# burn-research/OpenMEASURE

Measured on AMD Instinct MI355X. Metric: SPR fit+reconstruct throughput (GB/s snapshot matrix), higher is better.
Workload: dtype f64

## Files before the change

### include/spr_hip.h

```cpp
#ifndef SPR_HIP_H
#define SPR_HIP_H

#include <stddef.h>
#include <stdint.h>

#ifdef __cplusplus
extern "C" {
#endif

#define SPR_OK 0
#define SPR_E_INVALID (-1)
#define SPR_E_UNSUPPORTED (-2)
#define SPR_E_HIP (-3)
#define SPR_E_WORKSPACE (-4)

#define SPR_MAX_M 256
#define SPR_MAX_M_WIDE 512
#define SPR_MAX_R 128
#define SPR_MAX_R_STREAM 256
#define SPR_MAX_R_WIDE 1024

#define SPR_ABI_VERSION 5
int spr_abi_version(void);
const char *spr_last_error(void);
int spr_device_cus(int *out_cus);
int spr_upload_bytes(void *d_dst, const void *h_pinned_src, int64_t n_bytes, void *stream);
int spr_download_bytes(void *h_pinned_dst, const void *d_src, int64_t n_bytes, void *h_pinned_ticket, uint64_t ticket_value,
                       void *stream);
int spr_host_tridiag_vectors(const double *h_d, const double *h_e, int32_t m, const double *h_lam, int32_t r, double *h_Z,
                             int32_t iterations);
int spr_host_eig_top(const double *h_G, int32_t m, int32_t r, double *h_lam, double *h_V, void *fn_dsytrd, void *fn_dsterf,
                     void *fn_dormtr);
int spr_host_svd_top(const double *h_M, int32_t m, int32_t r, double *h_S, double *h_V, void *fn_dgebrd, void *fn_dbdsdc,
                     void *fn_dormbr);

size_t spr_stats_gram_workspace(int32_t m, int32_t n_features);
int spr_stats_gram_f64(const double *d_X, int64_t n_rows, int32_t m, int64_t ldx,
                       int64_t row0, int64_t n_points, int32_t n_features, int32_t center,
                       double *d_rowmean, void *d_workspace, size_t workspace_bytes, void *stream);
int spr_stats_gram_finalize_f64(int64_t n_rows, int32_t m, int64_t row0, int64_t n_points,
                                int32_t n_features, const void *d_workspace, size_t workspace_bytes,
                                double *d_fstats, double *d_gram, int32_t ldg, int32_t origin,
                                void *stream);
size_t spr_rowstats_workspace(int32_t n_features);
int spr_rowstats_f64(const double *d_X, int64_t n_rows, int32_t m, int64_t ldx, int64_t row0,
                     int64_t n_points, int32_t n_features, double *d_rowmean, double *d_fstats,
                     void *d_workspace, size_t workspace_bytes, void *stream);
size_t spr_gram_cross_workspace(int32_t m, int32_t n_features);
int spr_gram_cross_f64(const double *d_X, int64_t n_rows, int32_t m, int64_t ldx, int64_t row0,
                       int64_t n_points, int32_t n_features, int32_t center, double *d_rowmean,
                       double *d_gram, void *d_workspace, size_t workspace_bytes, void *stream);
int spr_rowmean_stats_f64(const double *d_rowmean, int64_t n_rows, int64_t row0, int64_t n_points,
                          int32_t n_features, double *d_fstats, void *d_workspace, size_t workspace_bytes,
                          void *stream);
int spr_gram_cross_pair_f64(const double *d_X, int64_t n_rows, int32_t col_a, int32_t col_b, int32_t w_b,
                            int32_t ldg, int64_t ldx, int64_t row0, int64_t n_points, int32_t n_features,
                            int32_t center, double *d_rowmean, double *d_gram, void *d_workspace,
                            size_t workspace_bytes, void *stream);

int32_t spr_spectrum_max_m(void);
int spr_spectrum_f64(const double *d_gram, const double *d_fstats_all, int32_t n_ranks,
                     int32_t n_features, int32_t m, int32_t scale_code, int32_t r, double *d_feat,
                     double *d_scale, double *d_inv_scale, double *d_lam, double *d_S, double *d_expvar,
                     double *d_V, double *d_W, double *d_Ar, double *d_info, void *stream);

int spr_gram_combine_f64(const double *d_gram, const double *d_fstats_all, int32_t n_ranks,
                         int32_t n_features, int32_t m, int32_t scale_code, double *d_G, double *d_feat,
                         double *d_scale, double *d_inv_scale, void *stream);

int spr_stats_gram_shifted_f64(const double *d_X, int64_t n_rows, int32_t m, int64_t ldx, int64_t row0,
                               int64_t n_points, int32_t n_features, const double *d_shift, double *d_rowsum,
                               void *d_workspace, size_t workspace_bytes, void *stream);
int spr_gram_shift_finish_f64(double *d_rowmean, const double *d_rowsum_b, int64_t n_rows, int32_t w_a, int32_t m,
                              double *d_gram, int32_t n_features, void *stream);

int spr_project_f64(const double *d_X, int64_t n_rows, int32_t m, int64_t ldx,
                    int64_t row0, int64_t n_points, int32_t n_features, int32_t center,
                    const double *d_inv_scale, const double *d_rowmean, const double *d_W, int32_t r,
                    double *d_Ur, int64_t ldu, int32_t accumulate, void *stream);

size_t spr_project_stream_workspace(int32_t m, int32_t r, int32_t x_is_f32);
int spr_project_stream_f64(const double *d_X, int64_t n_rows, int32_t m, int64_t ldx, int64_t row0,
                           int64_t n_points, int32_t n_features, int32_t center, const double *d_inv_scale,
                           const double *d_rowmean, const double *d_W, int32_t r, double *d_Ur, int64_t ldu,
                           void *d_workspace, size_t workspace_bytes, void *stream);

int32_t spr_project_norms_supported(int32_t m, int32_t r, int64_t n_rows, int64_t ldx, const void *d_X,
                                    int32_t x_is_f32);
int spr_project_norms_f64(const double *d_X, int64_t n_rows, int32_t m, int64_t ldx, int64_t row0,
                          int64_t n_points, int32_t n_features, int32_t center, const double *d_inv_scale,
                          const double *d_rowmean, const double *d_W, int32_t r, double *d_Ur, int64_t ldu,
                          double *d_rownorm2, void *stream);
int spr_project_stream_norms_f64(const double *d_X, int64_t n_rows, int32_t m, int64_t ldx, int64_t row0,
                                 int64_t n_points, int32_t n_features, int32_t center, const double *d_inv_scale,
                                 const double *d_rowmean, const double *d_W, int32_t r, double *d_Ur, int64_t ldu,
                                 double *d_rownorm2, void *d_workspace, size_t workspace_bytes, void *stream);

int spr_scale_rows_f64(const double *d_X, int64_t n_rows, int32_t m, int64_t ldx, int64_t row0,
                       int64_t n_points, int32_t n_features, const double *d_rowmean,
                       const double *d_inv_scale, double *d_X0, int64_t ldo, void *stream);
int spr_unscale_f64(const double *d_x0, int64_t n_rows, int64_t row0, int64_t n_points,
                    int32_t n_features, const double *d_rowmean, const double *d_scale,
                    const double *d_rowscale, double *d_x, void *stream);

size_t spr_feature_minmax_workspace(int32_t n_features);
int spr_feature_minmax_f64(const double *d_X, int64_t n_rows, int32_t m, int64_t ldx, int64_t row0,
                           int64_t n_points, int32_t n_features, double *d_minmax,
                           void *d_workspace, size_t workspace_bytes, void *stream);

int spr_feature_digit_hist_f64(const double *d_X, int64_t n_rows, int32_t m, int64_t ldx, int64_t row0,
                               int64_t n_points, int32_t n_features, const uint64_t *d_prefix, int32_t shift,
                               int32_t bits, int32_t two_targets, uint64_t *d_hist, void *stream);

size_t spr_colsums_workspace(int32_t m, int32_t n_features);
int spr_colsums_f64(const double *d_X, int64_t n_rows, int32_t m, int64_t ldx, int64_t row0,
                    int64_t n_points, int32_t n_features, const double *d_rowmean, double *d_out,
                    void *d_workspace, size_t workspace_bytes, void *stream);
int spr_fill_feature_f64(double *d_out, int64_t n_rows, int64_t row0, int64_t n_points, int32_t n_features,
                         const double *d_values, void *stream);

int spr_reconstruct_f64(const double *d_Ur, int64_t n_rows, int32_t r, int64_t ldu,
                        int64_t row0, int64_t n_points, int32_t n_features,
                        const double *d_rowmean, const double *d_scale, const double *d_rowscale,
                        const double *d_A, int32_t n_p, double *d_Xrec, int64_t ldo,
                        void *stream);
size_t spr_bound_sweep_workspace(int32_t n_p, int32_t n_features);
int spr_bound_sweep_f64(const double *d_Ur, int64_t n_rows, int32_t r, int64_t ldu, int64_t row0, int64_t n_points,
                        int32_t n_features, const double *d_rowmean, const double *d_scale, const double *d_limits,
                        const double *d_clamp, const double *d_G, int32_t n_p, double tol, int32_t k, double *d_out,
                        void *d_workspace, size_t workspace_bytes, void *stream);
int spr_bound_sweep_u32(const float *d_Ur, int64_t n_rows, int32_t r, int64_t ldu, int64_t row0, int64_t n_points,
                        int32_t n_features, const double *d_rowmean, const double *d_scale, const double *d_limits,
                        const double *d_clamp, const double *d_G, int32_t n_p, double tol, int32_t k, double *d_out,
                        void *d_workspace, size_t workspace_bytes, void *stream);
size_t spr_bound_sweep_batch_workspace(int32_t n_p, int32_t n_features);
int spr_bound_sweep_batch_f64(const double *d_Ur, int64_t n_rows, int32_t r, int64_t ldu, int64_t row0, int64_t n_points,
                              int32_t n_features, const double *d_rowmean, const double *d_scale, const double *d_limits,
                              const double *d_clamp, const double *d_G, int32_t n_p, double tol, int32_t k, double *d_out,
                              void *d_workspace, size_t workspace_bytes, void *stream);
int spr_bound_sweep_batch_u32(const float *d_Ur, int64_t n_rows, int32_t r, int64_t ldu, int64_t row0, int64_t n_points,
                              int32_t n_features, const double *d_rowmean, const double *d_scale, const double *d_limits,
                              const double *d_clamp, const double *d_G, int32_t n_p, double tol, int32_t k, double *d_out,
                              void *d_workspace, size_t workspace_bytes, void *stream);
size_t spr_encode_workspace(int32_t r, int32_t k, int32_t n_features);
int spr_encode_f64(const double *d_Ur, int64_t n_rows, int32_t r, int64_t ldu, const double *d_X, int32_t k, int64_t ldx,
                   int64_t row0, int64_t n_points, int32_t n_features, const double *d_rowmean, const double *d_scale,
                   double *d_A, void *d_workspace, size_t workspace_bytes, void *stream);
int spr_encode_x32(const double *d_Ur, int64_t n_rows, int32_t r, int64_t ldu, const float *d_X, int32_t k, int64_t ldx,
                   int64_t row0, int64_t n_points, int32_t n_features, const double *d_rowmean, const double *d_scale,
                   double *d_A, void *d_workspace, size_t workspace_bytes, void *stream);
int spr_encode_u32(const float *d_Ur, int64_t n_rows, int32_t r, int64_t ldu, const double *d_X, int32_t k, int64_t ldx,
                   int64_t row0, int64_t n_points, int32_t n_features, const double *d_rowmean, const double *d_scale,
                   double *d_A, void *d_workspace, size_t workspace_bytes, void *stream);
int spr_encode_x32_u32(const float *d_Ur, int64_t n_rows, int32_t r, int64_t ldu, const float *d_X, int32_t k, int64_t ldx,
                       int64_t row0, int64_t n_points, int32_t n_features, const double *d_rowmean, const double *d_scale,
                       double *d_A, void *d_workspace, size_t workspace_bytes, void *stream);
size_t spr_field_error_workspace(int32_t k, int32_t n_features);
int spr_field_error_f64(const double *d_Ur, int64_t n_rows, int32_t r, int64_t ldu, int64_t row0, int64_t n_points,
                        int32_t n_features, const double *d_rowmean, const double *d_scale, const double *d_A, int32_t k,
                        const double *d_Xtrue, int64_t ldx, double *d_out, void *d_workspace, size_t workspace_bytes,
                        void *stream);
int spr_field_error_x32(const double *d_Ur, int64_t n_rows, int32_t r, int64_t ldu, int64_t row0, int64_t n_points,
                        int32_t n_features, const double *d_rowmean, const double *d_scale, const double *d_A, int32_t k,
                        const float *d_Xtrue, int64_t ldx, double *d_out, void *d_workspace, size_t workspace_bytes,
                        void *stream);
int spr_field_error_u32(const float *d_Ur, int64_t n_rows, int32_t r, int64_t ldu, int64_t row0, int64_t n_points,
                        int32_t n_features, const double *d_rowmean, const double *d_scale, const double *d_A, int32_t k,
                        const double *d_Xtrue, int64_t ldx, double *d_out, void *d_workspace, size_t workspace_bytes,
                        void *stream);
int spr_field_error_x32_u32(const float *d_Ur, int64_t n_rows, int32_t r, int64_t ldu, int64_t row0, int64_t n_points,
                            int32_t n_features, const double *d_rowmean, const double *d_scale, const double *d_A, int32_t k,
                            const float *d_Xtrue, int64_t ldx, double *d_out, void *d_workspace, size_t workspace_bytes,
                            void *stream);
size_t spr_gappy_normal_workspace(int32_t r, int32_t k, int32_t n_features);
int spr_gappy_normal_f64(const double *d_Ur, int64_t n_rows, int32_t r, int64_t ldu, const double *d_X, int32_t k,
                         int64_t ldx, int64_t row0, int64_t n_points, int32_t n_features, const double *d_rowmean,
                         const double *d_scale, const uint8_t *d_mask, int64_t ldm, double *d_H, double *d_B,
                         double *d_nobs, void *d_workspace, size_t workspace_bytes, void *stream);
int spr_gappy_normal_x32(const double *d_Ur, int64_t n_rows, int32_t r, int64_t ldu, const float *d_X, int32_t k,
                         int64_t ldx, int64_t row0, int64_t n_points, int32_t n_features, const double *d_rowmean,
                         const double *d_scale, const uint8_t *d_mask, int64_t ldm, double *d_H, double *d_B,
                         double *d_nobs, void *d_workspace, size_t workspace_bytes, void *stream);
int spr_gappy_normal_u32(const float *d_Ur, int64_t n_rows, int32_t r, int64_t ldu, const double *d_X, int32_t k,
                         int64_t ldx, int64_t row0, int64_t n_points, int32_t n_features, const double *d_rowmean,
                         const double *d_scale, const uint8_t *d_mask, int64_t ldm, double *d_H, double *d_B,
                         double *d_nobs, void *d_workspace, size_t workspace_bytes, void *stream);
int spr_gappy_normal_x32_u32(const float *d_Ur, int64_t n_rows, int32_t r, int64_t ldu, const float *d_X, int32_t k,
                             int64_t ldx, int64_t row0, int64_t n_points, int32_t n_features, const double *d_rowmean,
                             const double *d_scale, const uint8_t *d_mask, int64_t ldm, double *d_H, double *d_B,
                             double *d_nobs, void *d_workspace, size_t workspace_bytes, void *stream);
size_t spr_gappy_fill_workspace(void);
int spr_gappy_rowfill_f64(double *d_X, int64_t n_rows, int32_t m, int64_t ldx, int64_t row0, const uint8_t *d_mask,
                          int64_t ldm, double *d_out, void *d_workspace, size_t workspace_bytes, void *stream);
int spr_gappy_rowfill_x32(float *d_X, int64_t n_rows, int32_t m, int64_t ldx, int64_t row0, const uint8_t *d_mask,
                          int64_t ldm, double *d_out, void *d_workspace, size_t workspace_bytes, void *stream);
int spr_gappy_fill_f64(const double *d_Ur, int64_t n_rows, int32_t r, int64_t ldu, double *d_X, int32_t m, int64_t ldx,
                       int64_t row0, int64_t n_points, int32_t n_features, const double *d_rowmean, const double *d_scale,
                       const double *d_A, const uint8_t *d_mask, int64_t ldm, double *d_out, void *d_workspace,
                       size_t workspace_bytes, void *stream);
int spr_gappy_fill_x32(const double *d_Ur, int64_t n_rows, int32_t r, int64_t ldu, float *d_X, int32_t m, int64_t ldx,
                       int64_t row0, int64_t n_points, int32_t n_features, const double *d_rowmean, const double *d_scale,
                       const double *d_A, const uint8_t *d_mask, int64_t ldm, double *d_out, void *d_workspace,
                       size_t workspace_bytes, void *stream);
int spr_gappy_fill_u32(const float *d_Ur, int64_t n_rows, int32_t r, int64_t ldu, double *d_X, int32_t m, int64_t ldx,
                       int64_t row0, int64_t n_points, int32_t n_features, const double *d_rowmean, const double *d_scale,
                       const double *d_A, const uint8_t *d_mask, int64_t ldm, double *d_out, void *d_workspace,
                       size_t workspace_bytes, void *stream);
int spr_gappy_fill_x32_u32(const float *d_Ur, int64_t n_rows, int32_t r, int64_t ldu, float *d_X, int32_t m, int64_t ldx,
                           int64_t row0, int64_t n_points, int32_t n_features, const double *d_rowmean,
                           const double *d_scale, const double *d_A, const uint8_t *d_mask, int64_t ldm, double *d_out,
                           void *d_workspace, size_t workspace_bytes, void *stream);
int spr_field_std_diag_f64(const double *d_Ur, int64_t n_rows, int32_t r, int64_t ldu, int64_t row0, int64_t n_points,
                           int32_t n_features, const double *d_scale, const double *d_rowscale, const double *d_S,
                           int32_t k, double *d_out, int64_t ldo, void *stream);
int spr_field_std_diag_u32(const float *d_Ur, int64_t n_rows, int32_t r, int64_t ldu, int64_t row0, int64_t n_points,
                           int32_t n_features, const double *d_scale, const double *d_rowscale, const double *d_S,
                           int32_t k, double *d_out, int64_t ldo, void *stream);
int spr_field_std_factor_f64(const double *d_Ur, int64_t n_rows, int32_t r, int64_t ldu, int64_t row0, int64_t n_points,
                             int32_t n_features, const double *d_scale, const double *d_rowscale, const double *d_L,
                             int32_t k, int32_t q, double *d_out, int64_t ldo, void *stream);
int spr_field_std_factor_u32(const float *d_Ur, int64_t n_rows, int32_t r, int64_t ldu, int64_t row0, int64_t n_points,
                             int32_t n_features, const double *d_scale, const double *d_rowscale, const double *d_L,
                             int32_t k, int32_t q, double *d_out, int64_t ldo, void *stream);
#define SPR_GP_MAX_M 800
#define SPR_GP_MATERN52 0
#define SPR_GP_MATERN32 1
#define SPR_GP_MATERN12 2
#define SPR_GP_RBF 3
size_t spr_gp_workspace(int32_t m, int32_t r);
int spr_gp_train_f64(const double *d_P0, int32_t m, int32_t d, int64_t ldp, const double *d_Y, int32_t r, int64_t ldy,
                     int32_t kernel, double *d_raw, double lr, int32_t max_iter, double tol, double *d_Kinv, double *d_alpha,
                     double *d_info, double *d_trace, void *d_workspace, size_t workspace_bytes, void *stream);
int spr_gp_predict_f64(const double *d_P0, int32_t m, int32_t d, int64_t ldp, const double *d_Pstar, int32_t n_p,
                       int64_t ldps, int32_t kernel, const double *d_raw, int32_t r, const double *d_Kinv,
                       const double *d_alpha, double *d_mean, double *d_var, void *stream);
#define SPR_GP_MAX_D 8
#define SPR_GP_FLAG_ARD 1
#define SPR_GP_FLAG_SCALE 2
size_t spr_gp_workspace_ard(int32_t m, int32_t d, int32_t r);
int spr_gp_train_ard_f64(const double *d_P0, int32_t m, int32_t d, int64_t ldp, const double *d_Y, int32_t r, int64_t ldy,
                         int32_t kernel, int32_t flags, double *d_raw, double lr, int32_t max_iter, double tol,
                         double *d_Kinv, double *d_alpha, double *d_info, double *d_trace, void *d_workspace,
                         size_t workspace_bytes, void *stream);
int spr_gp_predict_ard_f64(const double *d_P0, int32_t m, int32_t d, int64_t ldp, const double *d_Pstar, int32_t n_p,
                           int64_t ldps, int32_t kernel, int32_t flags, const double *d_raw, int32_t r, const double *d_Kinv,
                           const double *d_alpha, double *d_mean, double *d_var, void *stream);
int spr_field_unstage_f64(const double *d_stage, int32_t world, int32_t n_p, int64_t n_loc, double *d_out, int64_t ldo,
                          void *stream);
int spr_field_unstage_blocks_f64(const double *d_stage, int32_t world, int32_t n_p, int64_t n_max, const int64_t *d_layout,
                                 double *d_out, int64_t ldo, void *stream);

size_t spr_p2p_handle_bytes(void);
int spr_p2p_alloc(size_t n_bytes, int32_t kind, void **d_ptr, void *h_handle);
int spr_p2p_free(void *d_ptr);
int spr_p2p_open(const void *h_handle, void **d_mapped);
int spr_p2p_close(void *d_mapped);
int spr_p2p_device_id(char *h_buf, int32_t n_buf);
int spr_p2p_peer_access(const char *h_bus_id, int32_t *h_can);
int spr_p2p_signal(void *d_flag, uint64_t value, void *stream);
int spr_p2p_wait(void *d_flag, uint64_t value, void *stream);
int spr_p2p_flags_set(void *const *d_flags, int32_t n, uint64_t value, void *stream);
int spr_p2p_flags_wait(void *const *d_flags, int32_t n, uint64_t value, double timeout_s, void *d_status, void *stream);
int spr_p2p_copy(void *d_dst, const void *d_src, int64_t n_bytes, void *stream);
uint64_t spr_p2p_poison_bit(void);
int spr_field_gather_p2p(const double *d_field, int64_t ldo, int32_t n_p, int64_t first, int64_t n_loc, int32_t n_peers,
                         void *const *d_peer_field, void *const *d_release_flag, uint64_t release_value,
                         double release_timeout_s, void *const *d_peer_arrive_flag, uint64_t arrive_value,
                         void *const *d_pushed_flag, void *const *streams, void *d_status, void *d_ready_flag,
                         uint64_t ready_value);
int spr_field_gather_p2p_join(void *const *d_flags, int32_t n_flags, uint64_t arrive_value, double timeout_s, void *d_status,
                              void *stream);
int spr_field_gather_p2p_release(void *const *d_peer_release_flag, int32_t n_peers, uint64_t value, void *stream);

size_t spr_comm_unique_id_bytes(void);
int spr_comm_unique_id(void *h_id);
int spr_comm_init(const void *h_id, int32_t rank, int32_t world, void **comm);
int spr_comm_destroy(void *comm);
int spr_comm_info(void *comm, int32_t *rank, int32_t *world);
const char *spr_comm_library(void);
int spr_allreduce_f64(void *comm, double *d_buf, int64_t count, void *stream);
int spr_allreduce_i64(void *comm, int64_t *d_buf, int64_t count, void *stream);
int spr_allgather(void *comm, const void *d_send, void *d_recv, int64_t bytes_per_rank, void *stream);
size_t spr_fit_gram_pass_buffer(int32_t m, int32_t n_features, int32_t world);
size_t spr_fit_gram_pass_workspace(int32_t m, int32_t n_features, int64_t n_rows);
int spr_fit_gram_pass(void *comm, const void *d_X, int32_t x_is_f32, int64_t n_rows, int32_t m, int64_t ldx, int64_t row0,
                      int64_t n_points, int32_t n_features, int32_t scale_code, double *d_rowmean, double *d_buf,
                      size_t buf_bytes, double *d_G, double *d_feat, double *d_scale, double *d_inv_scale, void *d_workspace,
                      size_t workspace_bytes, void *stream);

#define SPR_QR_REC_LEN(r) ((r) + 3)
size_t spr_qr_workspace(int64_t n_rows);
size_t spr_qr_workspace_r(int64_t n_rows, int32_t r);
int32_t spr_qr_batch(void);
int spr_mask_rows_f64(double *d_Ur, int64_t n_rows, int32_t r, int64_t ldu,
                      const uint8_t *d_mask, void *stream);
int spr_qr_init_f64(const double *d_Ur, int64_t n_rows, int32_t r, int64_t ldu,
                    int64_t row0, double *d_nrm, double *d_rec, double *d_tau,
                    void *d_workspace, size_t workspace_bytes, void *stream);
int spr_qr_init_norms_f64(const double *d_Ur, int64_t n_rows, int32_t r, int64_t ldu, int64_t row0,
                          const double *d_nrm0, double *d_nrm, double *d_rec, double *d_tau,
                          void *d_workspace, size_t workspace_bytes, void *stream);
int spr_qr_step_f64(int64_t n_rows, int32_t r, int32_t step, const double *d_recs, int32_t n_rec,
                    const double *d_taus, int32_t n_tau, int32_t first, double *d_Q,
                    int64_t *d_piv, double *d_gap, double *d_ok, double *d_rec,
                    const double *d_xyz, int32_t xyz_dim, int64_t n_points, double d_min,
                    void *d_workspace, size_t workspace_bytes, void *stream);
int spr_qr_steps_f64(int64_t n_rows, int32_t r, int32_t step0, int32_t n_steps, int32_t first_exact,
                     const double *d_tau, double *d_Q, int64_t *d_piv, double *d_gap, double *d_ok, double *d_rec,
                     const double *d_xyz, int32_t xyz_dim, int64_t n_points, double d_min,
                     void *d_workspace, size_t workspace_bytes, void *stream);
int32_t spr_qr_epoch_supported(int32_t r, int64_t ldu, const void *d_Ur, int32_t u_is_f32, int64_t n_rows);
int32_t spr_qr_epoch_max_directions(int32_t r);
size_t spr_qr_pool_workspace(void);
int spr_qr_pool_build(const double *d_nrm_e, int64_t n_rows, double theta, int32_t *d_pool, int64_t cap,
                      int32_t *d_pool_n, void *d_workspace, size_t workspace_bytes, void *stream);
int spr_qr_epoch_sweep_f64(const double *d_Ur, int64_t n_rows, int32_t r, int64_t ldu, int64_t row0,
                           const double *d_Q, const int64_t *d_piv, int32_t j_e, int32_t j, int32_t j_mark,
                           double *d_nrm_e, double *d_nrm, const int32_t *d_pool, const int32_t *d_pool_n,
                           int64_t pool_n_host, double tau_floor, double *d_rec, double *d_tau,
                           void *d_workspace, size_t workspace_bytes, void *stream);
int spr_qr_exclude_f64(double *d_nrm, int64_t n_rows, int64_t row0, int64_t n_points,
                       const uint8_t *d_mask, const double *d_xyz, int32_t xyz_dim,
                       const int64_t *d_piv, int32_t nq, double d_min, void *stream);
int spr_qr_refresh_f64(const double *d_Ur, int64_t n_rows, int32_t r, int64_t ldu, int64_t row0,
                       const double *d_Q, const int64_t *d_piv, int32_t j0, int32_t nq,
                       double *d_nrm, double *d_rec, double *d_tau,
                       void *d_workspace, size_t workspace_bytes, void *stream);

int spr_measure_csr_f64(const int64_t *d_indptr, const int64_t *d_indices,
                        const double *d_vals, int32_t s, const double *d_Ur,
                        int64_t n_rows, int32_t r, int64_t ldu, int64_t row0,
                        const double *d_rowmean, const double *d_scale, int64_t n_points,
                        int32_t n_features, double *d_Theta, double *d_cnt, double *d_scl,
                        void *stream);

int spr_solve_ols_f64(const double *d_Theta, int32_t s, int32_t r, const double *d_cnt,
                      const double *d_scale, int32_t n_features, const double *d_y,
                      int32_t n_p, double *d_Ar, double *d_Ar_sigma, double *d_y0,
                      double *d_info, void *stream);

size_t spr_solve_ols_workspace(int32_t s, int32_t r, int32_t n_p);
int spr_solve_ols_wide_f64(const double *d_Theta, int32_t s, int32_t r, const double *d_cnt,
                           const double *d_scale, int32_t n_features, const double *d_y, int32_t n_p,
                           double *d_Ar, double *d_Ar_sigma, double *d_y0, double *d_info, void *d_workspace,
                           size_t workspace_bytes, void *stream);

int spr_solve_pinv_f64(const double *d_Theta, int32_t s, int32_t r, const double *d_cnt, int32_t s_cnt,
                       const double *d_scale, int32_t n_features, const double *d_y, int32_t n_p,
                       double rcond, double *d_Ar, double *d_Ar_sigma, double *d_y0, double *d_info,
                       void *stream);

size_t spr_solve_pinv_workspace(int32_t r, int32_t n_p);
int spr_solve_pinv_wide_f64(const double *d_Theta, int32_t s, int32_t r, const double *d_cnt, int32_t s_cnt,
                            const double *d_scale, int32_t n_features, const double *d_y, int32_t n_p,
                            double rcond, double *d_Ar, double *d_Ar_sigma, double *d_y0, double *d_info,
                            void *d_workspace, size_t workspace_bytes, void *stream);

size_t spr_assimilate_workspace(int32_t s, int32_t r, int32_t q, int32_t n_p);
int spr_assimilate_f64(const double *d_Theta, int32_t s, int32_t r, const double *d_cnt, const double *d_scale,
                       int32_t n_features, const double *d_y, int32_t n_p, const double *d_a0, const double *d_sigma,
                       const double *d_factor, int32_t q, double *d_Ar, double *d_Ar_std, double *d_F, double *d_z,
                       double *d_info, void *d_workspace, size_t workspace_bytes, void *stream);

int spr_synth_f64(double *d_X, int64_t n_rows, int32_t ncols, int64_t ldx, int64_t row0,
                  int64_t n_points, int32_t col0, const double *d_R, int32_t k, int32_t ldr,
                  double eps, uint64_t seed, void *stream);
int spr_synth_gather_f64(const int64_t *d_rows, int32_t n, int64_t n_points, int32_t col,
                         const double *d_R, int32_t k, int32_t ldr, double eps,
                         uint64_t seed, double *d_out, void *stream);

int spr_stats_gram_x32(const float *d_X, int64_t n_rows, int32_t m, int64_t ldx, int64_t row0,
                       int64_t n_points, int32_t n_features, int32_t center, double *d_rowmean,
                       void *d_workspace, size_t workspace_bytes, void *stream);
int spr_rowstats_x32(const float *d_X, int64_t n_rows, int32_t m, int64_t ldx, int64_t row0,
                     int64_t n_points, int32_t n_features, double *d_rowmean, double *d_fstats,
                     void *d_workspace, size_t workspace_bytes, void *stream);
int spr_gram_cross_x32(const float *d_X, int64_t n_rows, int32_t m, int64_t ldx, int64_t row0,
                       int64_t n_points, int32_t n_features, int32_t center, double *d_rowmean,
                       double *d_gram, void *d_workspace, size_t workspace_bytes, void *stream);
int spr_gram_cross_pair_x32(const float *d_X, int64_t n_rows, int32_t col_a, int32_t col_b, int32_t w_b,
                            int32_t ldg, int64_t ldx, int64_t row0, int64_t n_points, int32_t n_features,
                            int32_t center, double *d_rowmean, double *d_gram, void *d_workspace,
                            size_t workspace_bytes, void *stream);
int spr_project_x32(const float *d_X, int64_t n_rows, int32_t m, int64_t ldx, int64_t row0,
                    int64_t n_points, int32_t n_features, int32_t center, const double *d_inv_scale,
                    const double *d_rowmean, const double *d_W, int32_t r, float *d_Ur, int64_t ldu,
                    int32_t accumulate, void *stream);
int spr_project_x32_f64out(const float *d_X, int64_t n_rows, int32_t m, int64_t ldx, int64_t row0,
                           int64_t n_points, int32_t n_features, int32_t center, const double *d_inv_scale,
                           const double *d_rowmean, const double *d_W, int32_t r, double *d_Ur, int64_t ldu,
                           int32_t accumulate, void *stream);
int spr_project_x32_acc(const float *d_X, int64_t n_rows, int32_t m, int64_t ldx, int64_t row0,
                        int64_t n_points, int32_t n_features, int32_t center, const double *d_inv_scale,
                        const double *d_rowmean, const double *d_W, int32_t r, const double *d_acc_in,
                        int64_t lda, float *d_Ur, int64_t ldu, void *stream);
int spr_project_stream_x32(const float *d_X, int64_t n_rows, int32_t m, int64_t ldx, int64_t row0,
                           int64_t n_points, int32_t n_features, int32_t center, const double *d_inv_scale,
                           const double *d_rowmean, const double *d_W, int32_t r, float *d_Ur, int64_t ldu,
                           void *d_workspace, size_t workspace_bytes, void *stream);
int spr_project_stream_x32_f64out(const float *d_X, int64_t n_rows, int32_t m, int64_t ldx, int64_t row0,
                                  int64_t n_points, int32_t n_features, int32_t center, const double *d_inv_scale,
                                  const double *d_rowmean, const double *d_W, int32_t r, double *d_Ur, int64_t ldu,
                                  void *d_workspace, size_t workspace_bytes, void *stream);
int spr_project_norms_x32(const float *d_X, int64_t n_rows, int32_t m, int64_t ldx, int64_t row0,
                          int64_t n_points, int32_t n_features, int32_t center, const double *d_inv_scale,
                          const double *d_rowmean, const double *d_W, int32_t r, float *d_Ur, int64_t ldu,
                          double *d_rownorm2, void *stream);
int spr_project_norms_x32_f64out(const float *d_X, int64_t n_rows, int32_t m, int64_t ldx, int64_t row0,
                                 int64_t n_points, int32_t n_features, int32_t center, const double *d_inv_scale,
                                 const double *d_rowmean, const double *d_W, int32_t r, double *d_Ur, int64_t ldu,
                                 double *d_rownorm2, void *stream);
int spr_project_stream_norms_x32(const float *d_X, int64_t n_rows, int32_t m, int64_t ldx, int64_t row0,
                                 int64_t n_points, int32_t n_features, int32_t center, const double *d_inv_scale,
                                 const double *d_rowmean, const double *d_W, int32_t r, float *d_Ur, int64_t ldu,
                                 double *d_rownorm2, void *d_workspace, size_t workspace_bytes, void *stream);
int spr_project_stream_norms_x32_f64out(const float *d_X, int64_t n_rows, int32_t m, int64_t ldx, int64_t row0,
                                        int64_t n_points, int32_t n_features, int32_t center,
                                        const double *d_inv_scale, const double *d_rowmean, const double *d_W,
                                        int32_t r, double *d_Ur, int64_t ldu, double *d_rownorm2, void *d_workspace,
                                        size_t workspace_bytes, void *stream);
int spr_stats_gram_shifted_x32(const float *d_X, int64_t n_rows, int32_t m, int64_t ldx, int64_t row0,
                               int64_t n_points, int32_t n_features, const double *d_shift, double *d_rowsum,
                               void *d_workspace, size_t workspace_bytes, void *stream);
int spr_scale_rows_x32(const float *d_X, int64_t n_rows, int32_t m, int64_t ldx, int64_t row0,
                       int64_t n_points, int32_t n_features, const double *d_rowmean,
                       const double *d_inv_scale, double *d_X0, int64_t ldo, void *stream);
int spr_feature_minmax_x32(const float *d_X, int64_t n_rows, int32_t m, int64_t ldx, int64_t row0,
                           int64_t n_points, int32_t n_features, double *d_minmax,
                           void *d_workspace, size_t workspace_bytes, void *stream);
int spr_colsums_x32(const float *d_X, int64_t n_rows, int32_t m, int64_t ldx, int64_t row0,
                    int64_t n_points, int32_t n_features, const double *d_rowmean, double *d_out,
                    void *d_workspace, size_t workspace_bytes, void *stream);
int spr_feature_digit_hist_x32(const float *d_X, int64_t n_rows, int32_t m, int64_t ldx, int64_t row0,
                               int64_t n_points, int32_t n_features, const uint64_t *d_prefix, int32_t shift,
                               int32_t bits, int32_t two_targets, uint64_t *d_hist, void *stream);
int spr_synth_f32(float *d_X, int64_t n_rows, int32_t ncols, int64_t ldx, int64_t row0,
                  int64_t n_points, int32_t col0, const double *d_R, int32_t k, int32_t ldr,
                  double eps, uint64_t seed, void *stream);
int spr_reconstruct_u32(const float *d_Ur, int64_t n_rows, int32_t r, int64_t ldu, int64_t row0,
                        int64_t n_points, int32_t n_features, const double *d_rowmean,
                        const double *d_scale, const double *d_rowscale, const double *d_A, int32_t n_p,
                        double *d_Xrec, int64_t ldo, void *stream);
int spr_mask_rows_u32(float *d_Ur, int64_t n_rows, int32_t r, int64_t ldu,
                      const uint8_t *d_mask, void *stream);
int spr_qr_init_u32(const float *d_Ur, int64_t n_rows, int32_t r, int64_t ldu,
                    int64_t row0, double *d_nrm, double *d_rec, double *d_tau,
                    void *d_workspace, size_t workspace_bytes, void *stream);
int spr_qr_init_norms_u32(const float *d_Ur, int64_t n_rows, int32_t r, int64_t ldu, int64_t row0,
                          const double *d_nrm0, double *d_nrm, double *d_rec, double *d_tau,
                          void *d_workspace, size_t workspace_bytes, void *stream);
int spr_qr_epoch_sweep_u32(const float *d_Ur, int64_t n_rows, int32_t r, int64_t ldu, int64_t row0,
                           const double *d_Q, const int64_t *d_piv, int32_t j_e, int32_t j, int32_t j_mark,
                           double *d_nrm_e, double *d_nrm, const int32_t *d_pool, const int32_t *d_pool_n,
                           int64_t pool_n_host, double tau_floor, double *d_rec, double *d_tau,
                           void *d_workspace, size_t workspace_bytes, void *stream);
int spr_qr_refresh_u32(const float *d_Ur, int64_t n_rows, int32_t r, int64_t ldu, int64_t row0,
                       const double *d_Q, const int64_t *d_piv, int32_t j0, int32_t nq,
                       double *d_nrm, double *d_rec, double *d_tau,
                       void *d_workspace, size_t workspace_bytes, void *stream);
int spr_measure_csr_u32(const int64_t *d_indptr, const int64_t *d_indices, const double *d_vals,
                        int32_t s, const float *d_Ur, int64_t n_rows, int32_t r, int64_t ldu,
                        int64_t row0, const double *d_rowmean, const double *d_scale, int64_t n_points,
                        int32_t n_features, double *d_Theta, double *d_cnt, double *d_scl, void *stream);

#ifdef __cplusplus
}
#endif
#endif
```

### openmeasure_amd/_lib.py

```python
from __future__ import annotations

import ctypes as C
import os

_HERE = os.path.dirname(os.path.abspath(__file__))
LIB_PATH = os.environ.get('SPR_HIP_LIBRARY') or os.path.join(_HERE, 'libspr_hip.so')

SPR_ABI_VERSION = 5
SPR_MAX_M = 256
SPR_MAX_M_WIDE = 512
SPR_MAX_R = 128
SPR_MAX_R_STREAM = 256
SPR_MAX_R_WIDE = 1024
SPR_GP_MAX_M = 800
SPR_GP_MAX_D = 8

_i32, _i64, _u64, _sz = C.c_int32, C.c_int64, C.c_uint64, C.c_size_t
_p = C.c_void_p
_dbl = C.c_double

PROTOTYPES = {
    'spr_abi_version': (C.c_int, []),
    'spr_last_error': (C.c_char_p, []),
    'spr_device_cus': (C.c_int, [C.POINTER(C.c_int)]),
    'spr_upload_bytes': (C.c_int, [_p, _p, _i64, _p]),
    'spr_download_bytes': (C.c_int, [_p, _p, _i64, _p, _u64, _p]),
    'spr_host_tridiag_vectors': (C.c_int, [_p, _p, _i32, _p, _i32, _p, _i32]),
    'spr_host_eig_top': (C.c_int, [_p, _i32, _i32, _p, _p, _p, _p, _p]),
    'spr_host_svd_top': (C.c_int, [_p, _i32, _i32, _p, _p, _p, _p, _p]),
    'spr_stats_gram_workspace': (_sz, [_i32, _i32]),
    'spr_stats_gram_f64': (C.c_int, [_p, _i64, _i32, _i64, _i64, _i64, _i32, _i32, _p, _p, _sz, _p]),
    'spr_stats_gram_finalize_f64': (C.c_int, [_i64, _i32, _i64, _i64, _i32, _p, _sz, _p, _p, _i32, _i32, _p]),
    'spr_stats_gram_shifted_f64': (C.c_int, [_p, _i64, _i32, _i64, _i64, _i64, _i32, _p, _p, _p, _sz, _p]),
    'spr_gram_shift_finish_f64': (C.c_int, [_p, _p, _i64, _i32, _i32, _p, _i32, _p]),
    'spr_rowstats_workspace': (_sz, [_i32]),
    'spr_rowstats_f64': (C.c_int, [_p, _i64, _i32, _i64, _i64, _i64, _i32, _p, _p, _p, _sz, _p]),
    'spr_gram_cross_workspace': (_sz, [_i32, _i32]),
    'spr_gram_cross_f64': (C.c_int, [_p, _i64, _i32, _i64, _i64, _i64, _i32, _i32, _p, _p, _p, _sz, _p]),
    'spr_gram_cross_pair_f64': (C.c_int, [_p, _i64, _i32, _i32, _i32, _i32, _i64, _i64, _i64, _i32, _i32, _p, _p, _p, _sz, _p]),
    'spr_rowmean_stats_f64': (C.c_int, [_p, _i64, _i64, _i64, _i32, _p, _p, _sz, _p]),
    'spr_spectrum_max_m': (_i32, []),
    'spr_spectrum_f64': (C.c_int, [_p, _p, _i32, _i32, _i32, _i32, _i32, _p, _p, _p, _p, _p, _p, _p, _p, _p, _p, _p]),
    'spr_gram_combine_f64': (C.c_int, [_p, _p, _i32, _i32, _i32, _i32, _p, _p, _p, _p, _p]),
    'spr_project_f64': (C.c_int, [_p, _i64, _i32, _i64, _i64, _i64, _i32, _i32, _p, _p, _p, _i32, _p, _i64, _i32, _p]),
    'spr_project_norms_supported': (_i32, [_i32, _i32, _i64, _i64, _p, _i32]),
    'spr_project_norms_f64': (C.c_int, [_p, _i64, _i32, _i64, _i64, _i64, _i32, _i32, _p, _p, _p, _i32, _p, _i64, _p, _p]),
    'spr_project_stream_norms_f64': (C.c_int, [_p, _i64, _i32, _i64, _i64, _i64, _i32, _i32, _p, _p, _p, _i32, _p, _i64, _p, _p, _sz, _p]),
    'spr_project_stream_workspace': (_sz, [_i32, _i32, _i32]),
    'spr_project_stream_f64': (C.c_int, [_p, _i64, _i32, _i64, _i64, _i64, _i32, _i32, _p, _p, _p, _i32, _p, _i64, _p, _sz, _p]),
    'spr_scale_rows_f64': (C.c_int, [_p, _i64, _i32, _i64, _i64, _i64, _i32, _p, _p, _p, _i64, _p]),
    'spr_unscale_f64': (C.c_int, [_p, _i64, _i64, _i64, _i32, _p, _p, _p, _p, _p]),
    'spr_feature_minmax_workspace': (_sz, [_i32]),
    'spr_feature_minmax_f64': (C.c_int, [_p, _i64, _i32, _i64, _i64, _i64, _i32, _p, _p, _sz, _p]),
    'spr_feature_digit_hist_f64': (C.c_int, [_p, _i64, _i32, _i64, _i64, _i64, _i32, _p, _i32, _i32, _i32, _p, _p]),
    'spr_colsums_workspace': (_sz, [_i32, _i32]),
    'spr_colsums_f64': (C.c_int, [_p, _i64, _i32, _i64, _i64, _i64, _i32, _p, _p, _p, _sz, _p]),
    'spr_fill_feature_f64': (C.c_int, [_p, _i64, _i64, _i64, _i32, _p, _p]),
    'spr_reconstruct_f64': (C.c_int, [_p, _i64, _i32, _i64, _i64, _i64, _i32, _p, _p, _p, _p, _i32, _p, _i64, _p]),
    'spr_bound_sweep_workspace': (_sz, [_i32, _i32]),
    'spr_bound_sweep_f64': (C.c_int, [_p, _i64, _i32, _i64, _i64, _i64, _i32, _p, _p, _p, _p, _p, _i32, _dbl, _i32, _p, _p, _sz, _p]),
    'spr_bound_sweep_batch_workspace': (_sz, [_i32, _i32]),
    'spr_bound_sweep_batch_f64': (C.c_int, [_p, _i64, _i32, _i64, _i64, _i64, _i32, _p, _p, _p, _p, _p, _i32, _dbl, _i32, _p, _p, _sz, _p]),
    'spr_encode_workspace': (_sz, [_i32, _i32, _i32]),
    'spr_encode_f64': (C.c_int, [_p, _i64, _i32, _i64, _p, _i32, _i64, _i64, _i64, _i32, _p, _p, _p, _p, _sz, _p]),
    'spr_field_error_workspace': (_sz, [_i32, _i32]),
    'spr_field_error_f64': (C.c_int, [_p, _i64, _i32, _i64, _i64, _i64, _i32, _p, _p, _p, _i32, _p, _i64, _p, _p, _sz, _p]),
    'spr_gappy_normal_workspace': (_sz, [_i32, _i32, _i32]),
    'spr_gappy_normal_f64': (C.c_int, [_p, _i64, _i32, _i64, _p, _i32, _i64, _i64, _i64, _i32, _p, _p, _p, _i64, _p, _p, _p, _p, _sz, _p]),
    'spr_gappy_fill_workspace': (_sz, []),
    'spr_gappy_rowfill_f64': (C.c_int, [_p, _i64, _i32, _i64, _i64, _p, _i64, _p, _p, _sz, _p]),
    'spr_gappy_fill_f64': (C.c_int, [_p, _i64, _i32, _i64, _p, _i32, _i64, _i64, _i64, _i32, _p, _p, _p, _p, _i64, _p, _p, _sz, _p]),
    'spr_field_std_diag_f64': (C.c_int, [_p, _i64, _i32, _i64, _i64, _i64, _i32, _p, _p, _p, _i32, _p, _i64, _p]),
    'spr_field_std_factor_f64': (C.c_int, [_p, _i64, _i32, _i64, _i64, _i64, _i32, _p, _p, _p, _i32, _i32, _p, _i64, _p]),
    'spr_gp_workspace': (_sz, [_i32, _i32]),
    'spr_gp_train_f64': (C.c_int, [_p, _i32, _i32, _i64, _p, _i32, _i64, _i32, _p, _dbl, _i32, _dbl, _p, _p, _p, _p, _p, _sz, _p]),
    'spr_gp_predict_f64': (C.c_int, [_p, _i32, _i32, _i64, _p, _i32, _i64, _i32, _p, _i32, _p, _p, _p, _p, _p]),
    'spr_gp_workspace_ard': (_sz, [_i32, _i32, _i32]),
    'spr_gp_train_ard_f64': (C.c_int, [_p, _i32, _i32, _i64, _p, _i32, _i64, _i32, _i32, _p, _dbl, _i32, _dbl, _p, _p, _p, _p, _p, _sz, _p]),
    'spr_gp_predict_ard_f64': (C.c_int, [_p, _i32, _i32, _i64, _p, _i32, _i64, _i32, _i32, _p, _i32, _p, _p, _p, _p, _p]),
    'spr_field_unstage_f64': (C.c_int, [_p, _i32, _i32, _i64, _p, _i64, _p]),
    'spr_field_unstage_blocks_f64': (C.c_int, [_p, _i32, _i32, _i64, _p, _p, _i64, _p]),
    'spr_p2p_handle_bytes': (_sz, []),
    'spr_p2p_alloc': (C.c_int, [_sz, _i32, _p, _p]),
    'spr_p2p_free': (C.c_int, [_p]),
    'spr_p2p_open': (C.c_int, [_p, _p]),
    'spr_p2p_close': (C.c_int, [_p]),
    'spr_p2p_device_id': (C.c_int, [_p, _i32]),
    'spr_p2p_peer_access': (C.c_int, [_p, _p]),
    'spr_p2p_signal': (C.c_int, [_p, _u64, _p]),
    'spr_p2p_wait': (C.c_int, [_p, _u64, _p]),
    'spr_p2p_flags_set': (C.c_int, [_p, _i32, _u64, _p]),
    'spr_p2p_flags_wait': (C.c_int, [_p, _i32, _u64, _dbl, _p, _p]),
    'spr_p2p_copy': (C.c_int, [_p, _p, _i64, _p]),
    'spr_p2p_poison_bit': (_u64, []),
    'spr_field_gather_p2p': (C.c_int, [_p, _i64, _i32, _i64, _i64, _i32, _p, _p, _u64, _dbl, _p, _u64, _p, _p, _p, _p, _u64]),
    'spr_field_gather_p2p_join': (C.c_int, [_p, _i32, _u64, _dbl, _p, _p]),
    'spr_field_gather_p2p_release': (C.c_int, [_p, _i32, _u64, _p]),
    'spr_qr_workspace': (_sz, [_i64]),
    'spr_qr_workspace_r': (_sz, [_i64, _i32]),
    'spr_qr_batch': (_i32, []),
    'spr_mask_rows_f64': (C.c_int, [_p, _i64, _i32, _i64, _p, _p]),
    'spr_qr_init_f64': (C.c_int, [_p, _i64, _i32, _i64, _i64, _p, _p, _p, _p, _sz, _p]),
    'spr_qr_init_norms_f64': (C.c_int, [_p, _i64, _i32, _i64, _i64, _p, _p, _p, _p, _p, _sz, _p]),
    'spr_qr_step_f64': (C.c_int, [_i64, _i32, _i32, _p, _i32, _p, _i32, _i32, _p, _p, _p, _p, _p, _p, _i32, _i64, _dbl, _p, _sz, _p]),
    'spr_qr_steps_f64': (C.c_int, [_i64, _i32, _i32, _i32, _i32, _p, _p, _p, _p, _p, _p, _p, _i32, _i64, _dbl, _p, _sz, _p]),
    'spr_qr_epoch_supported': (_i32, [_i32, _i64, _p, _i32, _i64]),
    'spr_qr_epoch_max_directions': (_i32, [_i32]),
    'spr_qr_pool_workspace': (_sz, []),
    'spr_qr_pool_build': (C.c_int, [_p, _i64, _dbl, _p, _i64, _p, _p, _sz, _p]),
    'spr_qr_epoch_sweep_f64': (C.c_int, [_p, _i64, _i32, _i64, _i64, _p, _p, _i32, _i32, _i32, _p, _p, _p, _p, _i64, _dbl, _p, _p, _p, _sz, _p]),
    'spr_qr_exclude_f64': (C.c_int, [_p, _i64, _i64, _i64, _p, _p, _i32, _p, _i32, _dbl, _p]),
    'spr_qr_refresh_f64': (C.c_int, [_p, _i64, _i32, _i64, _i64, _p, _p, _i32, _i32, _p, _p, _p, _p, _sz, _p]),
    'spr_measure_csr_f64': (C.c_int, [_p, _p, _p, _i32, _p, _i64, _i32, _i64, _i64, _p, _p, _i64, _i32, _p, _p, _p, _p]),
    'spr_solve_ols_f64': (C.c_int, [_p, _i32, _i32, _p, _p, _i32, _p, _i32, _p, _p, _p, _p, _p]),
    'spr_solve_ols_workspace': (_sz, [_i32, _i32, _i32]),
    'spr_solve_ols_wide_f64': (C.c_int, [_p, _i32, _i32, _p, _p, _i32, _p, _i32, _p, _p, _p, _p, _p, _sz, _p]),
    'spr_solve_pinv_f64': (C.c_int, [_p, _i32, _i32, _p, _i32, _p, _i32, _p, _i32, _dbl, _p, _p, _p, _p, _p]),
    'spr_solve_pinv_workspace': (_sz, [_i32, _i32]),
    'spr_solve_pinv_wide_f64': (C.c_int, [_p, _i32, _i32, _p, _i32, _p, _i32, _p, _i32, _dbl, _p, _p, _p, _p, _p, _sz, _p]),
    'spr_assimilate_workspace': (_sz, [_i32, _i32, _i32, _i32]),
    'spr_assimilate_f64': (C.c_int, [_p, _i32, _i32, _p, _p, _i32, _p, _i32, _p, _p, _p, _i32, _p, _p, _p, _p, _p, _p, _sz, _p]),
    'spr_comm_unique_id_bytes': (_sz, []),
    'spr_comm_unique_id': (C.c_int, [_p]),
    'spr_comm_init': (C.c_int, [_p, _i32, _i32, _p]),
    'spr_comm_destroy': (C.c_int, [_p]),
    'spr_comm_info': (C.c_int, [_p, _p, _p]),
    'spr_comm_library': (C.c_char_p, []),
    'spr_allreduce_f64': (C.c_int, [_p, _p, _i64, _p]),
    'spr_allreduce_i64': (C.c_int, [_p, _p, _i64, _p]),
    'spr_allgather': (C.c_int, [_p, _p, _p, _i64, _p]),
    'spr_fit_gram_pass_buffer': (_sz, [_i32, _i32, _i32]),
    'spr_fit_gram_pass_workspace': (_sz, [_i32, _i32, _i64]),
    'spr_fit_gram_pass': (C.c_int, [_p, _p, _i32, _i64, _i32, _i64, _i64, _i64, _i32, _i32, _p, _p, _sz, _p, _p, _p, _p, _p, _sz, _p]),
    'spr_synth_f64': (C.c_int, [_p, _i64, _i32, _i64, _i64, _i64, _i32, _p, _i32, _i32, _dbl, _u64, _p]),
    'spr_synth_gather_f64': (C.c_int, [_p, _i32, _i64, _i32, _p, _i32, _i32, _dbl, _u64, _p, _p]),
}

_lib = None


class SprError(RuntimeError):
    """A libspr_hip.so call returned a negative status."""


PROTOTYPES['spr_project_x32_acc'] = (C.c_int, [_p, _i64, _i32, _i64, _i64, _i64, _i32, _i32, _p, _p, _p, _i32, _p, _i64, _p, _i64, _p])

for _f64, _x32 in (('spr_stats_gram_f64', 'spr_stats_gram_x32'), ('spr_stats_gram_shifted_f64', 'spr_stats_gram_shifted_x32'), ('spr_rowstats_f64', 'spr_rowstats_x32'),
                   ('spr_gram_cross_f64', 'spr_gram_cross_x32'), ('spr_gram_cross_pair_f64', 'spr_gram_cross_pair_x32'), ('spr_project_f64', 'spr_project_x32'),
                   ('spr_project_f64', 'spr_project_x32_f64out'),
                   ('spr_project_stream_f64', 'spr_project_stream_x32'),
                   ('spr_project_stream_f64', 'spr_project_stream_x32_f64out'),
                   ('spr_project_norms_f64', 'spr_project_norms_x32'),
                   ('spr_project_norms_f64', 'spr_project_norms_x32_f64out'),
                   ('spr_project_stream_norms_f64', 'spr_project_stream_norms_x32'),
                   ('spr_project_stream_norms_f64', 'spr_project_stream_norms_x32_f64out'),
                   ('spr_qr_init_norms_f64', 'spr_qr_init_norms_u32'),
                   ('spr_qr_epoch_sweep_f64', 'spr_qr_epoch_sweep_u32'),
                   ('spr_scale_rows_f64', 'spr_scale_rows_x32'), ('spr_feature_minmax_f64', 'spr_feature_minmax_x32'),
                   ('spr_colsums_f64', 'spr_colsums_x32'), ('spr_feature_digit_hist_f64', 'spr_feature_digit_hist_x32'),
                   ('spr_synth_f64', 'spr_synth_f32'), ('spr_reconstruct_f64', 'spr_reconstruct_u32'),
                   ('spr_bound_sweep_f64', 'spr_bound_sweep_u32'),
                   ('spr_bound_sweep_batch_f64', 'spr_bound_sweep_batch_u32'),
                   ('spr_encode_f64', 'spr_encode_x32'), ('spr_encode_f64', 'spr_encode_u32'),
                   ('spr_encode_f64', 'spr_encode_x32_u32'),
                   ('spr_field_error_f64', 'spr_field_error_x32'), ('spr_field_error_f64', 'spr_field_error_u32'),
                   ('spr_field_error_f64', 'spr_field_error_x32_u32'),
                   ('spr_gappy_normal_f64', 'spr_gappy_normal_x32'), ('spr_gappy_normal_f64', 'spr_gappy_normal_u32'),
                   ('spr_gappy_normal_f64', 'spr_gappy_normal_x32_u32'),
                   ('spr_gappy_rowfill_f64', 'spr_gappy_rowfill_x32'),
                   ('spr_gappy_fill_f64', 'spr_gappy_fill_x32'), ('spr_gappy_fill_f64', 'spr_gappy_fill_u32'),
                   ('spr_gappy_fill_f64', 'spr_gappy_fill_x32_u32'),
                   ('spr_field_std_diag_f64', 'spr_field_std_diag_u32'),
                   ('spr_field_std_factor_f64', 'spr_field_std_factor_u32'),
                   ('spr_mask_rows_f64', 'spr_mask_rows_u32'), ('spr_qr_init_f64', 'spr_qr_init_u32'),
                   ('spr_qr_refresh_f64', 'spr_qr_refresh_u32'), ('spr_measure_csr_f64', 'spr_measure_csr_u32')):
    PROTOTYPES[_x32] = PROTOTYPES[_f64]


def load():
    global _lib
    if _lib is not None:
        return _lib
    if not os.path.exists(LIB_PATH):
        raise RuntimeError(
            f'{LIB_PATH} is missing: build it with `make -C openmeasure_amd/csrc` '
            '(or __graft_entry__.build()). There is no CPU fallback for the SPR kernels.')
    import torch
    lib = C.CDLL(LIB_PATH, mode=C.RTLD_GLOBAL)
    for name, (res, args) in PROTOTYPES.items():
        fn = getattr(lib, name)
        fn.restype = res
        fn.argtypes = args
    have = lib.spr_abi_version()
    if have != SPR_ABI_VERSION:
        raise RuntimeError(f'{LIB_PATH} reports ABI version {have}, this binding was written for {SPR_ABI_VERSION}: '
                           'rebuild the library (make -C openmeasure_amd/csrc) or use the matching package')
    _lib = lib
    return lib


def check(rc, what=''):
    if rc == 0:
        return
    msg = load().spr_last_error().decode('utf-8', 'replace')
    kinds = {-1: ValueError, -2: NotImplementedError, -3: SprError, -4: MemoryError}
    raise kinds.get(rc, SprError)(f'{what or "libspr_hip"} failed (status {rc}): {msg}')
```

### openmeasure_amd/csrc/common.hpp

```cpp
#pragma once
#include <hip/hip_runtime.h>
#include <stdint.h>
#include <stdio.h>

#include "spr_hip.h"

typedef double f64x4 __attribute__((ext_vector_type(4)));
typedef double f64x2 __attribute__((ext_vector_type(2)));

void spr_set_error(const char *fmt, ...);

#define SPR_REQUIRE(cond, code, ...)      \
  do {                                    \
    if (!(cond)) {                        \
      spr_set_error(__VA_ARGS__);         \
      return (code);                      \
    }                                     \
  } while (0)

#define SPR_HIP_TRY(expr)                                                          \
  do {                                                                             \
    hipError_t e__ = (expr);                                                       \
    if (e__ != hipSuccess) {                                                       \
      spr_set_error("%s failed: %s (%s:%d)", #expr, hipGetErrorString(e__),       \
                    __FILE__, __LINE__);                                           \
      return SPR_E_HIP;                                                            \
    }                                                                              \
  } while (0)

#define SPR_LAUNCH_CHECK()                                                         \
  do {                                                                             \
    hipError_t e__ = hipGetLastError();                                            \
    if (e__ != hipSuccess) {                                                       \
      spr_set_error("kernel launch failed: %s (%s:%d)", hipGetErrorString(e__),   \
                    __FILE__, __LINE__);                                           \
      return SPR_E_HIP;                                                            \
    }                                                                              \
  } while (0)

int spr_cached_cus();

struct SegPlan {
  int64_t row0, n_rows, n_points;
  int32_t n_features;
  int32_t total_wg;
  int32_t chunk_rows;
};

__host__ __device__ inline void seg_range(const SegPlan &p, int f, int64_t &lo, int64_t &hi) {
  int64_t glo = (int64_t)f * p.n_points, ghi = glo + p.n_points;
  if (glo < p.row0) glo = p.row0;
  if (ghi > p.row0 + p.n_rows) ghi = p.row0 + p.n_rows;
  if (ghi < glo) ghi = glo;
  lo = glo - p.row0;
  hi = ghi - p.row0;
}

__host__ __device__ inline int seg_wgs(const SegPlan &p, int64_t rows) {
  if (rows <= 0) return 0;
  int64_t w = rows * (int64_t)p.total_wg / p.n_rows;
  int64_t chunks = (rows + p.chunk_rows - 1) / p.chunk_rows;
  if (w > chunks) w = chunks;
  if (w < 1) w = 1;
  return (int)w;
}

__host__ __device__ inline int seg_first_feature(const SegPlan &p) { return (int)(p.row0 / p.n_points); }
__host__ __device__ inline int seg_last_feature(const SegPlan &p) {
  int64_t f = (p.row0 + p.n_rows - 1) / p.n_points;
  if (f > p.n_features - 1) f = p.n_features - 1;
  return (int)f;
}

inline int seg_total_wgs(const SegPlan &p) {
  int tot = 0;
  for (int f = seg_first_feature(p); f <= seg_last_feature(p); ++f) {
    int64_t lo, hi;
    seg_range(p, f, lo, hi);
    tot += seg_wgs(p, hi - lo);
  }
  return tot;
}

__device__ inline bool seg_locate(const SegPlan &p, int b, int &f, int &wl, int &wpf, int &base,
                                  int64_t &lo, int64_t &hi) {
  int acc = 0;
  int f1 = seg_last_feature(p);
  for (int ff = seg_first_feature(p); ff <= f1; ++ff) {
    seg_range(p, ff, lo, hi);
    int w = seg_wgs(p, hi - lo);
    if (b < acc + w) {
      f = ff; wl = b - acc; wpf = w; base = acc;
      return true;
    }
    acc += w;
  }
  return false;
}

template <int CTRL>
__device__ inline double dpp_f64(double v) {
  union { double d; int i[2]; } a, b;
  a.d = v;
  b.i[0] = __builtin_amdgcn_update_dpp(0, a.i[0], CTRL, 0xF, 0xF, true);
  b.i[1] = __builtin_amdgcn_update_dpp(0, a.i[1], CTRL, 0xF, 0xF, true);
  return b.d;
}

template <int WIDTH>
__device__ inline double group_sum_t(double v) {
  if (WIDTH >= 2) v += dpp_f64<0xB1>(v);
  if (WIDTH >= 4) v += dpp_f64<0x4E>(v);
  if (WIDTH >= 8) v += dpp_f64<0x141>(v);
  if (WIDTH >= 16) v += dpp_f64<0x140>(v);
  if (WIDTH >= 32) v += __shfl_xor(v, 16, 64);
  if (WIDTH >= 64) v += __shfl_xor(v, 32, 64);
  return v;
}

__device__ inline double group_sum(double v, int width) {
  for (int o = width >> 1; o > 0; o >>= 1) v += __shfl_xor(v, o, 64);
  return v;
}

constexpr int spr_pow2_divisor_le64(int n) {
  int p = 1;
  while (p < 64 && n % (2 * p) == 0) p *= 2;
  return p;
}

inline int spr_round_mt(int m) {
  static const int sup[] = {1, 2, 3, 4, 6, 8, 12, 16};
  int need = (m + 15) / 16;
  for (int s : sup)
    if (s >= need) return s;
  return -1;
}
```

### openmeasure_amd/csrc/launch.hpp

```cpp
#pragma once
#include "common.hpp"

inline int spr_cus_or_default() {
  const int cus = spr_cached_cus();
  return cus > 0 ? cus : 256;
}

inline bool spr_layout_ok(int64_t row0, int64_t n_rows, int64_t n_points, int32_t n_features) {
  return n_points > 0 && n_features > 0 && row0 >= 0 && row0 + n_rows <= n_points * (int64_t)n_features;
}
#define SPR_REQUIRE_LAYOUT(name, row0, n_rows, n_points, n_features) \
  SPR_REQUIRE(spr_layout_ok(row0, n_rows, n_points, n_features), SPR_E_INVALID, "%s: bad feature layout", name)

inline SegPlan spr_make_plan(int64_t row0, int64_t n_rows, int64_t n_points, int32_t n_features, int32_t chunk_rows) {
  SegPlan plan;
  plan.row0 = row0; plan.n_rows = n_rows; plan.n_points = n_points; plan.n_features = n_features;
  plan.total_wg = 0; plan.chunk_rows = chunk_rows;
  return plan;
}

inline int spr_plan_grid(SegPlan &plan, int per_cu, int chunk_rows) {
  plan.total_wg = per_cu * spr_cus_or_default();
  plan.chunk_rows = chunk_rows;
  return seg_total_wgs(plan);
}

inline int spr_plan_grid(SegPlan &plan, int per_cu) { return spr_plan_grid(plan, per_cu, plan.chunk_rows); }

constexpr int spr_panel_per_cu(int mtr) { return mtr <= 1 ? 6 : mtr == 2 ? 4 : mtr == 3 ? 3 : mtr == 4 ? 2 : 1; }

#define SPR_REQUIRE_GRID(name, grid, max_slots) \
  SPR_REQUIRE((grid) > 0 && (grid) <= (max_slots), SPR_E_INVALID, "%s: grid of %d exceeds the workspace", name, grid)

template <typename T>
inline bool spr_pair_aligned(const T *p, int64_t cols, int64_t ld) {
  return (cols % 2 == 0) && (ld % 2 == 0) && ((reinterpret_cast<uintptr_t>(p) & (2 * sizeof(T) - 1)) == 0);
}

inline bool spr_rows_aligned16(const void *p, size_t row_bytes) {
  return row_bytes % 16 == 0 && (reinterpret_cast<uintptr_t>(p) & 15) == 0;
}

inline int spr_load_mode(bool pair_aligned, int r, int mtr) { return pair_aligned ? (r == 16 * mtr ? 2 : 1) : 0; }

#define SPR_RUNG_(N, ...) \
  case N: {               \
    constexpr int RUNG = N; \
    __VA_ARGS__;          \
  } break;
#define SPR_NO_RUNG_(name, r) \
  default: SPR_REQUIRE(false, SPR_E_UNSUPPORTED, "%s: no kernel for the padded width of r = %d", name, (int)(r));

#define SPR_DISPATCH_MT(sel, name, r, ...)                   \
  switch (sel) {                                                                                                  \
    SPR_RUNG_(1, __VA_ARGS__) SPR_RUNG_(2, __VA_ARGS__) SPR_RUNG_(3, __VA_ARGS__) SPR_RUNG_(4, __VA_ARGS__)       \
    SPR_RUNG_(6, __VA_ARGS__) SPR_RUNG_(8, __VA_ARGS__) SPR_NO_RUNG_(name, r)                                     \
  }
#define SPR_DISPATCH_POW2(sel, name, r, ...)                         \
  switch (sel) {                                                                                                  \
    SPR_RUNG_(1, __VA_ARGS__) SPR_RUNG_(2, __VA_ARGS__) SPR_RUNG_(4, __VA_ARGS__) SPR_RUNG_(8, __VA_ARGS__)       \
    SPR_NO_RUNG_(name, r)                                                                                         \
  }
#define SPR_DISPATCH_1TO8(sel, name, r, ...)                                 \
  switch (sel) {                                                                                                  \
    SPR_RUNG_(1, __VA_ARGS__) SPR_RUNG_(2, __VA_ARGS__) SPR_RUNG_(3, __VA_ARGS__) SPR_RUNG_(4, __VA_ARGS__)       \
    SPR_RUNG_(5, __VA_ARGS__) SPR_RUNG_(6, __VA_ARGS__) SPR_RUNG_(7, __VA_ARGS__) SPR_RUNG_(8, __VA_ARGS__)       \
    SPR_NO_RUNG_(name, r)                                                                                         \
  }

#define SPR_ENTRY(NAME, PARAMS, IMPL, ...) \
  extern "C" int NAME PARAMS { return IMPL(#NAME, __VA_ARGS__); }
```

### openmeasure_amd/csrc/project_ws.hip

```cpp
#include <type_traits>

#include "rowtile.hpp"
#include "launch.hpp"

namespace {

#ifndef WS_ABLATE
#define WS_ABLATE 0
#endif
constexpr int WS_WAVES = 8;
constexpr int WS_ROWS = 16 * WS_WAVES;

template <int RT> struct WsLds { static constexpr int NC = 16 * RT, LDW = NC; static_assert(RT % 2 == 0, "column tiles come in pairs"); };

template <typename TX> struct WsPiece;
template <> struct WsPiece<double> { f64x2 a, b; };
template <> struct WsPiece<float> { float x, y, z, w; };

template <int VEC, typename TX>
__device__ inline WsPiece<TX> ws_load(const TX *__restrict__ rp, int col0, int m) {
  WsPiece<TX> p;
  if constexpr (std::is_same<TX, double>::value) {
    if (VEC) {
      p.a = *reinterpret_cast<const f64x2 *>(rp + col0);
      p.b = *reinterpret_cast<const f64x2 *>(rp + col0 + 2);
    } else {
      p.a.x = rp[col0 < m ? col0 : 0];         p.a.y = rp[col0 + 1 < m ? col0 + 1 : 0];
      p.b.x = rp[col0 + 2 < m ? col0 + 2 : 0]; p.b.y = rp[col0 + 3 < m ? col0 + 3 : 0];
    }
  } else {
    if (VEC) {
      const float4 v = *reinterpret_cast<const float4 *>(rp + col0);
      p.x = v.x; p.y = v.y; p.z = v.z; p.w = v.w;
    } else {
      p.x = rp[col0 < m ? col0 : 0];         p.y = rp[col0 + 1 < m ? col0 + 1 : 0];
      p.z = rp[col0 + 2 < m ? col0 + 2 : 0]; p.w = rp[col0 + 3 < m ? col0 + 3 : 0];
    }
  }
  return p;
}

template <typename TX>
__device__ inline double ws_elem(const WsPiece<TX> &p, int t) {
  if constexpr (std::is_same<TX, double>::value) return t == 0 ? p.a.x : t == 1 ? p.a.y : t == 2 ? p.b.x : p.b.y;
  else return (double)(t == 0 ? p.x : t == 1 ? p.y : t == 2 ? p.z : p.w);
}

template <int MT, int RT, int VEC, typename TX, typename TU, bool NRM>
__global__ __launch_bounds__(WS_WAVES * 64) void project_ws_kernel(
    const TX *__restrict__ X, int64_t ldx, int m, int center_i, SegPlan plan, const double *__restrict__ inv_scale,
    const double *__restrict__ rowmean, const double *__restrict__ W, int r, TU *__restrict__ Ur, int64_t ldu,
    double *__restrict__ nrm2) {
  constexpr int K = 16 * MT, NJ = MT;
  constexpr int NC = WsLds<RT>::NC, LDW = WsLds<RT>::LDW;
  __shared__ double Wl[K * LDW];

  int f, wl, wpf, base;
  int64_t lo, hi;
  if (!seg_locate(plan, blockIdx.x, f, wl, wpf, base, lo, hi)) return;

  const int lane = threadIdx.x & 63;
  const int wave = __builtin_amdgcn_readfirstlane(threadIdx.x >> 6);
  const int li = lane & 15, kk = lane >> 4;
  const double isc = inv_scale[f];

  for (int e = threadIdx.x; e < K * NC; e += WS_WAVES * 64) {
    const int k = e / NC, c = e - k * NC;
    Wl[k * LDW + (c >> 5) * 32 + (c & 15) * 2 + ((c >> 4) & 1)] = (k < m && c < r) ? W[(int64_t)k * r + c] * isc : 0.0;
  }
  __syncthreads();
  double wbar[RT];
#pragma unroll
  for (int ct = 0; ct < RT; ++ct) {
    double sacc = 0.0;
    if (center_i != 0) {
      for (int k = kk; k < K; k += 4) sacc += Wl[k * LDW + (ct >> 1) * 32 + li * 2 + (ct & 1)];
      sacc += __shfl_xor(sacc, 16, 64);
      sacc += __shfl_xor(sacc, 32, 64);
    }
    wbar[ct] = sacc;
  }

  const int64_t nchunks = (hi - lo + WS_ROWS - 1) / WS_ROWS;
  int64_t c = wl;
  if (c >= nchunks) return;
  const double *wb = Wl + (4 * kk) * LDW + 2 * li;
  const double *wb_hi = wb + 128 * LDW;

  auto row_ptr = [&](int64_t cc) {
    int64_t row = lo + cc * WS_ROWS + 16 * wave + li;
    row = row < hi ? row : hi - 1;
    return X + row * ldx;
  };
  WsPiece<TX> areg[NJ];
  {
    const TX *rp = row_ptr(c);
#pragma unroll
    for (int j = 0; j < NJ; ++j) areg[j] = ws_load<VEC, TX>(rp, 16 * j + 4 * kk, m);
  }
  while (c < nchunks) {
    const int64_t cn = c + wpf;
    const TX *rpn = row_ptr(cn < nchunks ? cn : c);
    const int64_t blk0 = lo + c * WS_ROWS + 16 * wave;
    double mu[4];
#pragma unroll
    for (int i = 0; i < 4; ++i) {
      const int64_t rr = blk0 + kk + 4 * i;
      const double v = rowmean[rr < hi ? rr : hi - 1];
      mu[i] = center_i != 0 ? v : 0.0;
    }
    f64x4 acc[RT];
#pragma unroll
    for (int ct = 0; ct < RT; ++ct) acc[ct] = (f64x4){0.0, 0.0, 0.0, 0.0};
    f64x2 bcur[RT / 2], bnxt[RT / 2];
#pragma unroll
    for (int p = 0; p < RT / 2; ++p) bcur[p] = *reinterpret_cast<const f64x2 *>(wb + 32 * p);
#pragma unroll
    for (int j = 0; j < NJ; ++j) {
#pragma unroll
      for (int t = 0; t < 4; ++t) {
        const int sn = 4 * j + t + 1;
        const int jn = (sn >> 2) % NJ, tn = sn & 3;
        const double *wj = (jn < 8 ? wb : wb_hi) + (16 * (jn & 7) + tn) * LDW;
#pragma unroll
        for (int p = 0; p < RT / 2; ++p) bnxt[p] = *reinterpret_cast<const f64x2 *>(wj + 32 * p);
        const double a = ws_elem<TX>(areg[j], t);
#pragma unroll
        for (int p = 0; p < RT / 2; ++p) {
#if WS_ABLATE == 1
          asm volatile("" ::"v"(a), "v"(bcur[p].x), "v"(bcur[p].y));
#else
          acc[2 * p] = __builtin_amdgcn_mfma_f64_16x16x4f64(a, bcur[p].x, acc[2 * p], 0, 0, 0);
          acc[2 * p + 1] = __builtin_amdgcn_mfma_f64_16x16x4f64(a, bcur[p].y, acc[2 * p + 1], 0, 0, 0);
#endif
        }
        if (t == 3) areg[j] = ws_load<VEC, TX>(rpn, 16 * j + 4 * kk, m);
        __builtin_amdgcn_sched_group_barrier(0x100, RT / 2, 0);
        __builtin_amdgcn_sched_group_barrier(0x008, RT, 0);
        __builtin_amdgcn_sched_barrier(0);
#pragma unroll
        for (int p = 0; p < RT / 2; ++p) bcur[p] = bnxt[p];
      }
    }
    {
      const bool full = (blk0 + 16 <= hi) && (r == NC);
      TU *up = Ur + (blk0 + kk) * ldu + li;
      double q[4] = {0.0, 0.0, 0.0, 0.0};
#pragma unroll
      for (int ct = 0; ct < RT; ++ct) {
        const double s[4] = {acc[ct].x - mu[0] * wbar[ct], acc[ct].y - mu[1] * wbar[ct],
                             acc[ct].z - mu[2] * wbar[ct], acc[ct].w - mu[3] * wbar[ct]};
        if (NRM) {
#pragma unroll
          for (int i = 0; i < 4; ++i) { const double v = (double)(TU)s[i]; q[i] = fma(v, v, q[i]); }
        }
        if (full) {
#pragma unroll
          for (int i = 0; i < 4; ++i) up[4 * i * ldu + 16 * ct] = (TU)s[i];
        } else if (16 * ct + li < r) {
#pragma unroll
          for (int i = 0; i < 4; ++i)
            if (blk0 + kk + 4 * i < hi) up[4 * i * ldu + 16 * ct] = (TU)s[i];
        }
      }
      if (NRM) {
#pragma unroll
        for (int i = 0; i < 4; ++i) {
          const double t = group_sum_t<16>(q[i]);
          if (li == i && blk0 + kk + 4 * i < hi) nrm2[blk0 + kk + 4 * i] = t;
        }
      }
    }
    c = cn;
  }
}

template <int MT, int RT, typename TX, typename TU>
int ws_launch(const TX *X, int64_t n_rows, int32_t m, int64_t ldx, int64_t row0, int64_t n_points, int32_t n_features,
              int center, const double *inv_scale, const double *rowmean, const double *W, int32_t r, TU *Ur,
              int64_t ldu, int accumulate, double *nrm2, hipStream_t st) {
  SegPlan plan = spr_make_plan(row0, n_rows, n_points, n_features, WS_ROWS);
  static const int narrow_per_cu = [] { const char *e = getenv("SPR_WS_WG_PER_CU"); const int v = e ? atoi(e) : 2; return v >= 1 && v <= 4 ? v : 2; }();
  const int grid = spr_plan_grid(plan, MT <= 4 ? narrow_per_cu : 1);
  const bool vec = (m == 16 * MT) && spr_rows_aligned16(X, sizeof(TX) * ldx);
  if (!vec) return SPR_E_UNSUPPORTED;
  if (nrm2)
    hipLaunchKernelGGL((project_ws_kernel<MT, RT, 1, TX, TU, true>), dim3(grid), dim3(WS_WAVES * 64), 0, st, X, ldx, (int)m,
                       center, plan, inv_scale, rowmean, W, (int)r, Ur, ldu, nrm2);
  else
    hipLaunchKernelGGL((project_ws_kernel<MT, RT, 1, TX, TU, false>), dim3(grid), dim3(WS_WAVES * 64), 0, st, X, ldx, (int)m,
                       center, plan, inv_scale, rowmean, W, (int)r, Ur, ldu, nrm2);
  SPR_LAUNCH_CHECK();
  return SPR_OK;
}

}

#include "project_ws.hpp"

template <typename TX, typename TU>
int spr_project_ws(const TX *d_X, int64_t n_rows, int32_t m, int64_t ldx, int64_t row0, int64_t n_points,
                   int32_t n_features, int32_t center, const double *d_inv_scale, const double *d_rowmean,
                   const double *d_W, int32_t r, TU *d_Ur, int64_t ldu, int32_t accumulate, double *d_rownorm2,
                   hipStream_t st) {
  if (accumulate) return SPR_E_UNSUPPORTED;
  const int mt = spr_round_mt(m);
  const int need = (r + 15) / 16;
  const int rt = need <= 2 ? 2 : need <= 4 ? 4 : 0;
#define WS(MTV, RTV)                                                                                             \
  if (mt == MTV && rt == RTV)                                                                                    \
    return ws_launch<MTV, RTV, TX, TU>(d_X, n_rows, m, ldx, row0, n_points, n_features, center, d_inv_scale,   \
                                        d_rowmean, d_W, r, d_Ur, ldu, accumulate, d_rownorm2, st)
#ifdef PROJ_WS_LAB
  WS(16, 4);
#else
  WS(4, 2); WS(4, 4); WS(8, 2); WS(8, 4); WS(12, 2); WS(12, 4); WS(16, 2); WS(16, 4);
#endif
#undef WS
  return SPR_E_UNSUPPORTED;
}

template int spr_project_ws<double, double>(const double *, int64_t, int32_t, int64_t, int64_t, int64_t, int32_t, int32_t,
                                            const double *, const double *, const double *, int32_t, double *, int64_t,
                                            int32_t, double *, hipStream_t);
#ifndef PROJ_WS_LAB
template int spr_project_ws<float, float>(const float *, int64_t, int32_t, int64_t, int64_t, int64_t, int32_t, int32_t,
                                          const double *, const double *, const double *, int32_t, float *, int64_t,
                                          int32_t, double *, hipStream_t);
template int spr_project_ws<float, double>(const float *, int64_t, int32_t, int64_t, int64_t, int64_t, int32_t, int32_t,
                                           const double *, const double *, const double *, int32_t, double *, int64_t,
                                           int32_t, double *, hipStream_t);
#endif
```

### openmeasure_amd/csrc/stats_gram.hip

```cpp
#include <stdlib.h>

#include <type_traits>

#include "rowtile.hpp"
#include "launch.hpp"

#ifndef GRAM_UNIT_PAIRING
#define GRAM_UNIT_PAIRING 1
#endif
#ifndef GRAM_ABLATE
#define GRAM_ABLATE 0
#endif
#if GRAM_ABLATE == 1
#define GRAM_MFMA(a, b, c) ({ asm volatile("" ::"v"(a), "v"(b)); (c); })
#else
#define GRAM_MFMA(a, b, c) __builtin_amdgcn_mfma_f64_16x16x4f64((a), (b), (c), 0, 0, 0)
#endif

namespace {

template <int MT>
struct GramShape {
  static constexpr int MPAD = 16 * MT;
  static constexpr int MP = MPAD + ((MT % 2 == 0) ? 16 : 0);
  static constexpr int T = MT * (MT + 1) / 2;
  static constexpr int NU = (MT + 1) / 2;
};

template <int MT> struct GramCfg;
template <> struct GramCfg<1>  { static constexpr int NW = 8,  R = 64, KS = 8; static constexpr bool DBUF = true; static constexpr int LPRMAX = 16; };
template <> struct GramCfg<2>  { static constexpr int NW = 8,  R = 32, KS = 8; static constexpr bool DBUF = true; static constexpr int LPRMAX = 16; };
template <> struct GramCfg<3>  { static constexpr int NW = 8,  R = 64, KS = 4; static constexpr bool DBUF = true; static constexpr int LPRMAX = 16; };
#ifndef GRAM4_R
#define GRAM4_R 64
#define GRAM4_LPR 8
#endif
template <> struct GramCfg<4>  { static constexpr int NW = 8,  R = GRAM4_R, KS = 4; static constexpr bool DBUF = true; static constexpr int LPRMAX = GRAM4_LPR; };
template <> struct GramCfg<6>  { static constexpr int NW = 12, R = 48, KS = 4; static constexpr bool DBUF = true; static constexpr int LPRMAX = 16; };
template <> struct GramCfg<8>  { static constexpr int NW = 8,  R = 32, KS = 2; static constexpr bool DBUF = true; static constexpr int LPRMAX = 16; };
template <> struct GramCfg<12> { static constexpr int NW = 12, R = 24, KS = 2; static constexpr bool DBUF = false; static constexpr int LPRMAX = 32; };
#ifndef GRAM_DBUF16
#define GRAM_DBUF16 false
#endif
template <> struct GramCfg<16> { static constexpr int NW = 8,  R = 32, KS = 1; static constexpr bool DBUF = GRAM_DBUF16; static constexpr int LPRMAX = 16; };

template <int MT> struct GramOut { static constexpr int KSO = (GramCfg<MT>::KS >= 4) ? 1 : GramCfg<MT>::KS; };

constexpr int tri_index(int mt, int ti, int tj) { return ti * mt - ti * (ti - 1) / 2 + (tj - ti); }

template <int MT>
__device__ inline void tile_coords(int idx, int &ti, int &tj) {
  ti = 0;
  while (ti < MT - 1 && idx >= MT - ti) { idx -= MT - ti; ++ti; }
  tj = ti + idx;
  if (tj > MT - 1) tj = MT - 1;
}

template <int MT, int U, int VEC, typename TX>
__device__ inline void gram_wave(const TX *__restrict__ X, int64_t ldx, int m, int center,
                                 int64_t lo, int64_t hi, int wl, int wpf, int ks, int wave, int lane,
                                 double *__restrict__ lds0, double *__restrict__ lds1,
                                 double *__restrict__ rowmean, double *__restrict__ stat_part,
                                 double *__restrict__ slab, double *__restrict__ rowsum) {
  using S = GramShape<MT>;
  using C = GramCfg<MT>;
  constexpr int R = C::R, KS = C::KS, NW = C::NW, MP = S::MP, T = S::T;
  constexpr int KROWS = R / KS, KSTEPS = KROWS / 4;
  constexpr int RA = U, RB = MT - 1 - U;
  constexpr int NA = MT - RA;
  constexpr int NB = (RB != RA) ? MT - RB : 0;
  static_assert(KROWS % 4 == 0, "k slice must be a multiple of the MFMA depth");
  using RT = RowTile<MT, R, MP, NW, C::LPRMAX, TX>;

  f64x4 accA[NA];
  f64x4 accB[NB > 0 ? NB : 1];
#pragma unroll
  for (int j = 0; j < NA; ++j) accA[j] = (f64x4){0.0, 0.0, 0.0, 0.0};
#pragma unroll
  for (int j = 0; j < NB; ++j) accB[j] = (f64x4){0.0, 0.0, 0.0, 0.0};

  RowStats st;
  st.init();
  RT tile;

  const int64_t nchunks = (hi - lo + R - 1) / R;
  int64_t c = wl;
  const double *mean_in = rowmean;
  tile.template load<VEC>(X, ldx, m, lo + c * R, hi, wave, lane, mean_in);
  tile.template center_store<true>(lds0, m, center, lo + c * R, hi, wave, lane, rowmean, &st, rowsum);
  int64_t cn = c + wpf;
  int64_t nrow0 = (cn < nchunks) ? lo + cn * R : hi;
  tile.template load<VEC>(X, ldx, m, nrow0, hi, wave, lane, mean_in);
  int buf = 0;
  const int frag = (lane >> 4) * MP + (lane & 15) + ks * KROWS * MP + RA * 16;
  while (c < nchunks) {
    double *cur = buf ? lds1 : lds0;
    double *nxt = buf ? lds0 : lds1;
    const int64_t c2 = cn + wpf;
    const int64_t n2row0 = (c2 < nchunks) ? lo + c2 * R : hi;
    __syncthreads();
    const double *p = cur + frag;
    if constexpr (C::DBUF) {
      double op[2][NA];
#pragma unroll
      for (int j = 0; j < NA; ++j) op[0][j] = p[16 * j];
#pragma unroll
      for (int k = 0; k < KSTEPS; ++k) {
        if (k + 1 < KSTEPS) {
#pragma unroll
          for (int j = 0; j < NA; ++j) op[(k + 1) & 1][j] = p[(k + 1) * 4 * MP + 16 * j];
        }
#pragma unroll
        for (int j = 0; j < NA; ++j)
          accA[j] = GRAM_MFMA(op[k & 1][0], op[k & 1][j], accA[j]);
#pragma unroll
        for (int j = 0; j < NB; ++j)
          accB[j] = GRAM_MFMA(op[k & 1][RB - RA], op[k & 1][RB - RA + j], accB[j]);
#pragma unroll
        for (int it = 0; it < RT::IT; ++it)
          if (GRAM_ABLATE != 2 && (it * KSTEPS) / RT::IT == k) {
            if (GRAM_ABLATE == 3) tile.raw_store_pass(it, nxt, m, nrow0, hi, wave, lane);
            else tile.template center_store_pass<true>(it, nxt, m, center, nrow0, hi, wave, lane, rowmean, &st, rowsum);
            tile.template load_pass<VEC>(it, X, ldx, m, n2row0, hi, wave, lane, mean_in);
          }
      }
    } else {
#pragma unroll
      for (int k = 0; k < KSTEPS; ++k) {
        double op[NA];
#pragma unroll
        for (int j = 0; j < NA; ++j) op[j] = p[k * 4 * MP + 16 * j];
#pragma unroll
        for (int j = 0; j < NA; ++j)
          accA[j] = GRAM_MFMA(op[0], op[j], accA[j]);
#pragma unroll
        for (int j = 0; j < NB; ++j)
          accB[j] = GRAM_MFMA(op[RB - RA], op[RB - RA + j], accB[j]);
#pragma unroll
        for (int it = 0; it < RT::IT; ++it)
          if (GRAM_ABLATE != 2 && (it * KSTEPS) / RT::IT == k) {
            if (GRAM_ABLATE == 3) tile.raw_store_pass(it, nxt, m, nrow0, hi, wave, lane);
            else tile.template center_store_pass<true>(it, nxt, m, center, nrow0, hi, wave, lane, rowmean, &st, rowsum);
            tile.template load_pass<VEC>(it, X, ldx, m, n2row0, hi, wave, lane, mean_in);
          }
      }
    }
    buf ^= 1;
    c = cn;
    cn = c2;
    nrow0 = n2row0;
  }

  constexpr int KSO = GramOut<MT>::KSO;
  if constexpr (KSO != KS) {
    static_assert((size_t)T * 256 <= (size_t)2 * R * MP, "tile staging must fit the panel buffers");
    double *red = lds0 + lane;
    for (int s = KS - 1; s >= 1; --s) {
      __syncthreads();
      if (ks == s) {
#pragma unroll
        for (int j = 0; j < NA; ++j) {
          double *tp = red + tri_index(MT, RA, RA + j) * 256;
          tp[0] = accA[j].x; tp[64] = accA[j].y; tp[128] = accA[j].z; tp[192] = accA[j].w;
        }
#pragma unroll
        for (int j = 0; j < NB; ++j) {
          double *tp = red + tri_index(MT, RB, RB + j) * 256;
          tp[0] = accB[j].x; tp[64] = accB[j].y; tp[128] = accB[j].z; tp[192] = accB[j].w;
        }
      }
      __syncthreads();
      if (ks == s - 1) {
#pragma unroll
        for (int j = 0; j < NA; ++j) {
          const double *tp = red + tri_index(MT, RA, RA + j) * 256;
          accA[j].x += tp[0]; accA[j].y += tp[64]; accA[j].z += tp[128]; accA[j].w += tp[192];
        }
#pragma unroll
        for (int j = 0; j < NB; ++j) {
          const double *tp = red + tri_index(MT, RB, RB + j) * 256;
          accB[j].x += tp[0]; accB[j].y += tp[64]; accB[j].z += tp[128]; accB[j].w += tp[192];
        }
      }
    }
  }
  if (KSO == KS || ks == 0) {
    double *sp = slab + ((int64_t)blockIdx.x * KSO + (KSO == KS ? ks : 0)) * T * 256 + lane;
#pragma unroll
    for (int j = 0; j < NA; ++j) {
      double *tp = sp + (int64_t)tri_index(MT, RA, RA + j) * 256;
      tp[0] = accA[j].x; tp[64] = accA[j].y; tp[128] = accA[j].z; tp[192] = accA[j].w;
    }
#pragma unroll
    for (int j = 0; j < NB; ++j) {
      double *tp = sp + (int64_t)tri_index(MT, RB, RB + j) * 256;
      tp[0] = accB[j].x; tp[64] = accB[j].y; tp[128] = accB[j].z; tp[192] = accB[j].w;
    }
  }
  if ((lane % RT::LPR) == 0) {
    double *q = stat_part + ((int64_t)blockIdx.x * RT::ROWS_PER_IT + wave * RT::RPW + lane / RT::LPR) * 3;
    q[0] = st.cnt; q[1] = st.mean(); q[2] = st.m2();
  }
}

__device__ inline void chan_merge(double &n, double &mu, double &m2, double nb, double mb, double sb) {
  if (nb > 0.0) {
    const double tot = n + nb, d = mb - mu;
    mu += d * nb / tot;
    m2 += sb + d * d * n * nb / tot;
    n = tot;
  }
}

template <int MT, int U, typename TX, bool EXT, bool SUMS>
__device__ inline void gram_wave_own(const TX *__restrict__ X, int64_t ldx, int64_t lo, int64_t hi, int wl, int wpf, int ks,
                                     int wave, int lane, double *__restrict__ lds0, double *__restrict__ lds1,
                                     double *__restrict__ rowmean, double *__restrict__ slab, double *__restrict__ rowsum) {
  using S = GramShape<MT>;
  using C = GramCfg<MT>;
  constexpr int R = C::R, KS = C::KS, NW = C::NW, MP = S::MP, T = S::T;
  constexpr int KROWS = R / KS, KSTEPS = KROWS / 4;
  constexpr int RA = U, RB = MT - 1 - U;
  constexpr int NA = MT - RA;
  constexpr int NB = (RB != RA) ? MT - RB : 0;
  using RT = RowTile<MT, R, MP, NW, C::LPRMAX, TX>;

  f64x4 accA[NA];
  f64x4 accB[NB > 0 ? NB : 1];
#pragma unroll
  for (int j = 0; j < NA; ++j) accA[j] = (f64x4){0.0, 0.0, 0.0, 0.0};
#pragma unroll
  for (int j = 0; j < NB; ++j) accB[j] = (f64x4){0.0, 0.0, 0.0, 0.0};

  RT tile;
  const int64_t nchunks = (hi - lo + R - 1) / R;
  const int64_t lane_off = (int64_t)(wave * RT::RPW + lane / RT::LPR) * ldx;
  auto base_of = [&](int64_t row0) { return X + row0 * ldx; };
  int64_t c = wl;
  int64_t crow0 = lo + c * R;
#pragma unroll
  for (int it = 0; it < RT::IT; ++it) tile.template load_pass_own<EXT>(it, base_of(crow0), ldx, lane_off, hi - crow0, wave, lane, rowmean, crow0);
  if (crow0 + R <= hi) {
#pragma unroll
    for (int it = 0; it < RT::IT; ++it) tile.template center_store_own<true, EXT, SUMS>(it, lds0, crow0, hi - crow0, wave, lane, rowmean, rowsum);
  } else {
#pragma unroll
    for (int it = 0; it < RT::IT; ++it) tile.template center_store_own<false, EXT, SUMS>(it, lds0, crow0, hi - crow0, wave, lane, rowmean, rowsum);
  }
  int64_t cn = c + wpf;
  int64_t nrow0 = (cn < nchunks) ? lo + cn * R : hi;
#pragma unroll
  for (int it = 0; it < RT::IT; ++it) tile.template load_pass_own<EXT>(it, base_of(nrow0 < hi ? nrow0 : lo), ldx, lane_off, hi - nrow0, wave, lane, rowmean, nrow0 < hi ? nrow0 : lo);
  int buf = 0;
  const int frag = (lane >> 4) * MP + (lane & 15) + ks * KROWS * MP + RA * 16;
  while (c < nchunks) {
    double *cur = buf ? lds1 : lds0;
    double *nxt = buf ? lds0 : lds1;
    const int64_t c2 = cn + wpf;
    const int64_t n2row0 = (c2 < nchunks) ? lo + c2 * R : hi;
    const TX *n2base = base_of(n2row0 < hi ? n2row0 : lo);
    const bool nfull = nrow0 + R <= hi;
    if (GRAM_ABLATE != 4) __syncthreads();
    const double *p = cur + frag;
    auto stage = [&](auto full_tag, int k) {
      constexpr bool FULL = decltype(full_tag)::value;
#pragma unroll
      for (int it = 0; it < RT::IT; ++it)
        if ((it * KSTEPS) / RT::IT == k) {
          tile.template center_store_own<FULL, EXT, SUMS>(it, nxt, nrow0, hi - nrow0, wave, lane, rowmean, rowsum);
          tile.template load_pass_own<EXT>(it, n2base, ldx, lane_off, hi - n2row0, wave, lane, rowmean, n2row0 < hi ? n2row0 : lo);
        }
    };
    if constexpr (C::DBUF) {
      double op[2][NA];
#pragma unroll
      for (int j = 0; j < NA; ++j) op[0][j] = p[16 * j];
#pragma unroll
      for (int k = 0; k < KSTEPS; ++k) {
        if (k + 1 < KSTEPS) {
#pragma unroll
          for (int j = 0; j < NA; ++j) op[(k + 1) & 1][j] = p[(k + 1) * 4 * MP + 16 * j];
        }
#pragma unroll
        for (int j = 0; j < NA; ++j) accA[j] = GRAM_MFMA(op[k & 1][0], op[k & 1][j], accA[j]);
#pragma unroll
        for (int j = 0; j < NB; ++j) accB[j] = GRAM_MFMA(op[k & 1][RB - RA], op[k & 1][RB - RA + j], accB[j]);
        if (nfull) stage(std::true_type{}, k); else stage(std::false_type{}, k);
      }
    } else {
#pragma unroll
      for (int k = 0; k < KSTEPS; ++k) {
        double op[NA];
#pragma unroll
        for (int j = 0; j < NA; ++j) op[j] = p[k * 4 * MP + 16 * j];
#pragma unroll
        for (int j = 0; j < NA; ++j) accA[j] = GRAM_MFMA(op[0], op[j], accA[j]);
#pragma unroll
        for (int j = 0; j < NB; ++j) accB[j] = GRAM_MFMA(op[RB - RA], op[RB - RA + j], accB[j]);
        if (nfull) stage(std::true_type{}, k); else stage(std::false_type{}, k);
      }
    }
    buf ^= 1;
    c = cn;
    cn = c2;
    nrow0 = n2row0;
  }
  double *sp = slab + ((int64_t)blockIdx.x * KS + ks) * T * 256 + lane;
#pragma unroll
  for (int j = 0; j < NA; ++j) {
    double *tp = sp + (int64_t)tri_index(MT, RA, RA + j) * 256;
    tp[0] = accA[j].x; tp[64] = accA[j].y; tp[128] = accA[j].z; tp[192] = accA[j].w;
  }
#pragma unroll
  for (int j = 0; j < NB; ++j) {
    double *tp = sp + (int64_t)tri_index(MT, RB, RB + j) * 256;
    tp[0] = accB[j].x; tp[64] = accB[j].y; tp[128] = accB[j].z; tp[192] = accB[j].w;
  }
}

template <int MT, typename TX, bool EXT, bool SUMS>
__global__ __launch_bounds__(GramCfg<MT>::NW * 64) void stats_gram_own_kernel(
    const TX *__restrict__ X, int64_t ldx, SegPlan plan, double *__restrict__ rowmean, double *__restrict__ slab,
    double *__restrict__ rowsum) {
  using S = GramShape<MT>;
  using C = GramCfg<MT>;
  constexpr int NU = S::NU;
  __shared__ double lds[2][C::R * S::MP];
  int f, wl, wpf, base;
  int64_t lo, hi;
  if (!seg_locate(plan, blockIdx.x, f, wl, wpf, base, lo, hi)) return;
  const int lane = threadIdx.x & 63;
  const int wave = __builtin_amdgcn_readfirstlane(threadIdx.x >> 6);
  const int ks = wave / NU;
  const int unit = (GRAM_UNIT_PAIRING && NU == 8 && C::KS == 1) ? ((wave < 4) ? wave : 11 - wave) : wave % NU;
#define GRAM_UNIT(UV)                                                                                          \
  case UV:                                                                                                     \
    if constexpr (UV < NU)                                                                                     \
      gram_wave_own<MT, UV, TX, EXT, SUMS>(X, ldx, lo, hi, wl, wpf, ks, wave, lane, lds[0], lds[1], rowmean, slab, rowsum); \
    break;
  switch (unit) {
    GRAM_UNIT(0) GRAM_UNIT(1) GRAM_UNIT(2) GRAM_UNIT(3) GRAM_UNIT(4) GRAM_UNIT(5) GRAM_UNIT(6) GRAM_UNIT(7)
    default: break;
  }
#undef GRAM_UNIT
}

constexpr int RS_THREADS = 1024;
__global__ __launch_bounds__(RS_THREADS) void gram_rowmean_stats_kernel(const double *__restrict__ rowmean, SegPlan plan,
                                                                        int slots_per_wg, double *__restrict__ stat_part) {
  __shared__ double sn[RS_THREADS / 64], smu[RS_THREADS / 64], sm2[RS_THREADS / 64];
  int f, wl, wpf, base;
  int64_t lo, hi;
  if (!seg_locate(plan, blockIdx.x, f, wl, wpf, base, lo, hi)) return;
  const int lane = threadIdx.x & 63, wave = threadIdx.x >> 6;
  RowStats st;
  st.init();
  const int64_t step = (int64_t)wpf * RS_THREADS;
  int64_t row = lo + (int64_t)wl * RS_THREADS + threadIdx.x;
  for (; row + 3 * step < hi; row += 4 * step) {
    const double a = rowmean[row], b = rowmean[row + step], c = rowmean[row + 2 * step], d = rowmean[row + 3 * step];
    st.push(a, true); st.push(b, true); st.push(c, true); st.push(d, true);
  }
  for (; row < hi; row += step) st.push(rowmean[row], true);
  double n = st.cnt, mu = st.mean(), m2 = st.m2();
  for (int o = 32; o > 0; o >>= 1) {
    const double on = __shfl_down(n, o, 64), om = __shfl_down(mu, o, 64), os = __shfl_down(m2, o, 64);
    chan_merge(n, mu, m2, on, om, os);
  }
  if (lane == 0) { sn[wave] = n; smu[wave] = mu; sm2[wave] = m2; }
  __syncthreads();
  double *q = stat_part + (int64_t)blockIdx.x * slots_per_wg * 3;
  if (threadIdx.x == 0) {
    n = 0.0; mu = 0.0; m2 = 0.0;
    for (int w = 0; w < RS_THREADS / 64; ++w) chan_merge(n, mu, m2, sn[w], smu[w], sm2[w]);
    q[0] = n; q[1] = mu; q[2] = m2;
  }
  for (int e = 3 + threadIdx.x; e < slots_per_wg * 3; e += RS_THREADS) q[e] = 0.0;
}

template <int MT, int VEC, typename TX>
__global__ __launch_bounds__(GramCfg<MT>::NW * 64) void stats_gram_kernel(
    const TX *__restrict__ X, int64_t ldx, int m, int center_i, SegPlan plan,
    double *__restrict__ rowmean, double *__restrict__ stat_part, double *__restrict__ slab, double *__restrict__ rowsum) {
  using S = GramShape<MT>;
  using C = GramCfg<MT>;
  constexpr int NU = S::NU;
  static_assert(NU * C::KS == C::NW, "waves = units x k slices");
  __shared__ double lds[2][C::R * S::MP];

  int f, wl, wpf, base;
  int64_t lo, hi;
  if (!seg_locate(plan, blockIdx.x, f, wl, wpf, base, lo, hi)) return;

  const int lane = threadIdx.x & 63;
  const int wave = __builtin_amdgcn_readfirstlane(threadIdx.x >> 6);
  const int unit = wave % NU, ks = wave / NU;
#define GRAM_UNIT(UV)                                                                                        \
  case UV:                                                                                                   \
    if constexpr (UV < NU)                                                                                   \
      gram_wave<MT, UV, VEC, TX>(X, ldx, m, center_i, lo, hi, wl, wpf, ks, wave, lane, lds[0],    \
                        lds[1], rowmean, stat_part, slab, rowsum);                                           \
    break;
  switch (unit) {
    GRAM_UNIT(0) GRAM_UNIT(1) GRAM_UNIT(2) GRAM_UNIT(3) GRAM_UNIT(4) GRAM_UNIT(5) GRAM_UNIT(6) GRAM_UNIT(7)
    default: break;
  }
#undef GRAM_UNIT
}

template <int MT>
__global__ __launch_bounds__(1024) void gram_finalize_kernel(
    const double *__restrict__ slab, const double *__restrict__ stat_part, int m, SegPlan plan,
    int slots_per_wg, double *__restrict__ gram, double *__restrict__ fstats, int ldg, int origin) {
  constexpr int T = GramShape<MT>::T;
  constexpr int KS = GramOut<MT>::KSO;
  __shared__ double red[4][256];
  const int f = blockIdx.y;
  const int tile = blockIdx.x;
  int base = 0, wpf = 0;
  {
    int acc = 0;
    const int f0 = seg_first_feature(plan), f1 = seg_last_feature(plan);
    for (int ff = f0; ff <= f1; ++ff) {
      int64_t lo, hi;
      seg_range(plan, ff, lo, hi);
      const int w = seg_wgs(plan, hi - lo);
      if (ff == f) { base = acc; wpf = w; }
      acc += w;
    }
  }
  int ti, tj;
  tile_coords<MT>(tile, ti, tj);
  const int e = threadIdx.x & 255, g = threadIdx.x >> 8;
  const int np = wpf * KS;
  const double *sp = slab + ((int64_t)base * KS * T + tile) * 256 + e;
  const int64_t stride = (int64_t)T * 256;
  double s0 = 0.0, s1 = 0.0, s2 = 0.0, s3 = 0.0;
  int p = g;
  for (; p + 12 < np; p += 16) {
    s0 += sp[p * stride];
    s1 += sp[(p + 4) * stride];
    s2 += sp[(p + 8) * stride];
    s3 += sp[(p + 12) * stride];
  }
  for (; p < np; p += 4) s0 += sp[p * stride];
  red[g][e] = (s0 + s1) + (s2 + s3);
  __syncthreads();
  if (g == 0) {
    const double sum = (red[0][e] + red[1][e]) + (red[2][e] + red[3][e]);
    const int l = e & 63, reg = e >> 6;
    const int gi = ti * 16 + (l >> 4) + 4 * reg, gj = tj * 16 + (l & 15);
    if (gi < m && gj < m) {
      double *G = gram + (int64_t)f * ldg * ldg + (int64_t)origin * ldg + origin;
      G[(int64_t)gi * ldg + gj] = sum;
      if (ti != tj) G[(int64_t)gj * ldg + gi] = sum;
    }
  }
  if (tile == 0) {
    __syncthreads();
    double n = 0.0, mu = 0.0, m2 = 0.0;
    const double *q = stat_part + (int64_t)base * slots_per_wg * 3;
    const int tot_slots = wpf * slots_per_wg;
    for (int pp = threadIdx.x; pp < tot_slots; pp += 1024) chan_merge(n, mu, m2, q[3 * pp], q[3 * pp + 1], q[3 * pp + 2]);
    double *sn = &red[0][0], *smu = &red[1][0], *sm2 = &red[2][0];
    for (int o = 32; o > 0; o >>= 1) {
      const double on = __shfl_down(n, o, 64), om = __shfl_down(mu, o, 64), os = __shfl_down(m2, o, 64);
      chan_merge(n, mu, m2, on, om, os);
    }
    const int w = threadIdx.x >> 6;
    if ((threadIdx.x & 63) == 0) { sn[w] = n; smu[w] = mu; sm2[w] = m2; }
    __syncthreads();
    if (threadIdx.x == 0) {
      n = 0.0; mu = 0.0; m2 = 0.0;
      for (int ww = 0; ww < 16; ++ww) chan_merge(n, mu, m2, sn[ww], smu[ww], sm2[ww]);
      fstats[3 * f] = n; fstats[3 * f + 1] = mu; fstats[3 * f + 2] = m2;
    }
  }
}

template <int MT>
int occupancy_wgs() {
  static int cached = 0;
  if (cached) return cached;
  int per_cu = 0;
  if (hipOccupancyMaxActiveBlocksPerMultiprocessor(&per_cu, stats_gram_kernel<MT, 2, double>, GramCfg<MT>::NW * 64, 0) != hipSuccess ||
      per_cu < 1)
    per_cu = 1;
  if (per_cu > 4) per_cu = 4;
  cached = per_cu * spr_cus_or_default();
  return cached;
}

template <int MT>
SegPlan make_plan(int64_t n_rows, int64_t row0, int64_t n_points, int32_t n_features) {
  SegPlan p;
  p.row0 = row0; p.n_rows = n_rows; p.n_points = n_points; p.n_features = n_features;
  p.total_wg = occupancy_wgs<MT>();
  p.chunk_rows = GramCfg<MT>::R;
  return p;
}

template <int MT>
size_t workspace_bytes(int32_t n_features) {
  using RT = RowTile<MT, GramCfg<MT>::R, GramShape<MT>::MP, GramCfg<MT>::NW, GramCfg<MT>::LPRMAX>;
  const int64_t max_grid = (int64_t)occupancy_wgs<MT>() + n_features;
  return (size_t)max_grid * GramCfg<MT>::KS * GramShape<MT>::T * 256 * sizeof(double) +
         (size_t)max_grid * RT::ROWS_PER_IT * 3 * sizeof(double);
}

template <int MT, typename TX>
int launch(const TX *X, int64_t n_rows, int32_t m, int64_t ldx, int64_t row0, int64_t n_points,
           int32_t n_features, int center, double *rowmean, void *ws, size_t ws_bytes, hipStream_t st,
           double *rowsum = nullptr) {
  SPR_REQUIRE(ws_bytes >= workspace_bytes<MT>(n_features), SPR_E_WORKSPACE,
              "spr_stats_gram_f64: workspace %zu < %zu", ws_bytes, workspace_bytes<MT>(n_features));
  SPR_REQUIRE(!rowsum || center == 2, SPR_E_INVALID, "spr_stats_gram: row sums are an output of centre mode 2 only");
  SegPlan plan = make_plan<MT>(n_rows, row0, n_points, n_features);
  const int grid = seg_total_wgs(plan);
  const int64_t max_grid = (int64_t)occupancy_wgs<MT>() + n_features;
  SPR_REQUIRE(grid >= 1 && grid <= max_grid, SPR_E_INVALID, "spr_stats_gram_f64: bad grid %d", grid);
  double *slab = static_cast<double *>(ws);
  double *stat_part = slab + (size_t)max_grid * GramCfg<MT>::KS * GramShape<MT>::T * 256;
  const int lm = spr_load_mode(spr_pair_aligned(X, m, ldx), m, MT);
#define SG_LAUNCH(LM)                                                                                         \
  hipLaunchKernelGGL((stats_gram_kernel<MT, LM, TX>), dim3(grid), dim3(GramCfg<MT>::NW * 64), 0, st, X, ldx, (int)m, \
                     center, plan, rowmean, stat_part, slab, rowsum)
  using RTL = RowTile<MT, GramCfg<MT>::R, GramShape<MT>::MP, GramCfg<MT>::NW, GramCfg<MT>::LPRMAX, TX>;
  static const bool own_on = [] { const char *e = getenv("SPR_GRAM_OWN"); return !(e && e[0] == '0'); }();
  if (MT >= 8 && lm == 2 && (center == 1 || center == 2) && own_on && spr_rows_aligned16(X, sizeof(TX) * ldx)) {
    if constexpr (MT >= 8) {
      if (center == 1)
        hipLaunchKernelGGL((stats_gram_own_kernel<MT, TX, false, false>), dim3(grid), dim3(GramCfg<MT>::NW * 64), 0, st, X, ldx,
                           plan, rowmean, slab, rowsum);
      else if (!rowsum)
        hipLaunchKernelGGL((stats_gram_own_kernel<MT, TX, true, false>), dim3(grid), dim3(GramCfg<MT>::NW * 64), 0, st, X, ldx,
                           plan, rowmean, slab, rowsum);
      else
        hipLaunchKernelGGL((stats_gram_own_kernel<MT, TX, true, true>), dim3(grid), dim3(GramCfg<MT>::NW * 64), 0, st, X, ldx,
                           plan, rowmean, slab, rowsum);
      SPR_LAUNCH_CHECK();
      hipLaunchKernelGGL(gram_rowmean_stats_kernel, dim3(grid), dim3(RS_THREADS), 0, st, rowmean, plan, (int)RTL::ROWS_PER_IT,
                         stat_part);
      SPR_LAUNCH_CHECK();
      return SPR_OK;
    }
  }
  if (lm == 2) SG_LAUNCH(2);
  else if (lm == 1) SG_LAUNCH(1);
  else SG_LAUNCH(0);
#undef SG_LAUNCH
  SPR_LAUNCH_CHECK();
  return SPR_OK;
}

template <int MT>
int launch_finalize(int64_t n_rows, int32_t m, int64_t row0, int64_t n_points, int32_t n_features,
                    double *fstats, double *gram, int ldg, int origin, const void *ws, size_t ws_bytes,
                    hipStream_t st) {
  using RT = RowTile<MT, GramCfg<MT>::R, GramShape<MT>::MP, GramCfg<MT>::NW, GramCfg<MT>::LPRMAX>;
  SPR_REQUIRE(ws_bytes >= workspace_bytes<MT>(n_features), SPR_E_WORKSPACE,
              "spr_stats_gram_finalize_f64: workspace %zu < %zu", ws_bytes, workspace_bytes<MT>(n_features));
  SegPlan plan = make_plan<MT>(n_rows, row0, n_points, n_features);
  const int64_t max_grid = (int64_t)occupancy_wgs<MT>() + n_features;
  const double *slab = static_cast<const double *>(ws);
  const double *stat_part = slab + (size_t)max_grid * GramCfg<MT>::KS * GramShape<MT>::T * 256;
  hipLaunchKernelGGL(gram_finalize_kernel<MT>, dim3(GramShape<MT>::T, n_features), dim3(1024), 0, st, slab,
                     stat_part, (int)m, plan, (int)RT::ROWS_PER_IT, gram, fstats, ldg, origin);
  SPR_LAUNCH_CHECK();
  return SPR_OK;
}

int check_args(const char *who, const void *X, int64_t n_rows, int32_t m, int64_t ldx, int64_t row0,
               int64_t n_points, int32_t n_features) {
  SPR_REQUIRE(X != nullptr, SPR_E_INVALID, "%s: X is NULL", who);
  SPR_REQUIRE(n_rows > 0 && m > 0 && ldx >= m, SPR_E_INVALID, "%s: bad shape n_rows=%lld m=%d ldx=%lld", who,
              (long long)n_rows, m, (long long)ldx);
  SPR_REQUIRE(n_points > 0 && n_features > 0 && row0 >= 0, SPR_E_INVALID, "%s: bad feature layout", who);
  SPR_REQUIRE(row0 + n_rows <= n_points * (int64_t)n_features, SPR_E_INVALID,
              "%s: rows [%lld,%lld) exceed n_points*n_features=%lld", who, (long long)row0,
              (long long)(row0 + n_rows), (long long)(n_points * (int64_t)n_features));
  SPR_REQUIRE(m <= SPR_MAX_M, SPR_E_UNSUPPORTED, "%s: m=%d > %d not built", who, m, SPR_MAX_M);
  return SPR_OK;
}

}

#define GRAM_DISPATCH_M(mt, CALL)            \
  switch (mt) {                              \
    case 1: CALL(1); break;                  \
    case 2: CALL(2); break;                  \
    case 3: CALL(3); break;                  \
    case 4: CALL(4); break;                  \
    case 6: CALL(6); break;                  \
    case 8: CALL(8); break;                  \
    case 12: CALL(12); break;                \
    case 16: CALL(16); break;                \
    default: break;                          \
  }

extern "C" size_t spr_stats_gram_workspace(int32_t m, int32_t n_features) {
  if (m <= 0 || m > SPR_MAX_M || n_features <= 0) return 0;
  size_t out = 0;
#define WS_CALL(MTV) out = workspace_bytes<MTV>(n_features)
  GRAM_DISPATCH_M(spr_round_mt(m), WS_CALL)
#undef WS_CALL
  return out;
}

extern "C" int spr_stats_gram_f64(const double *d_X, int64_t n_rows, int32_t m, int64_t ldx, int64_t row0,
                                  int64_t n_points, int32_t n_features, int32_t center, double *d_rowmean,
                                  void *d_workspace, size_t workspace_bytes_, void *stream) {
  int rc = check_args("spr_stats_gram_f64", d_X, n_rows, m, ldx, row0, n_points, n_features);
  if (rc != SPR_OK) return rc;
  SPR_REQUIRE(d_rowmean && d_workspace, SPR_E_INVALID, "spr_stats_gram_f64: NULL output/workspace");
  rc = SPR_E_UNSUPPORTED;
#define RUN_CALL(MTV)                                                                                \
  rc = launch<MTV>(d_X, n_rows, m, ldx, row0, n_points, n_features, center, d_rowmean, d_workspace, \
                   workspace_bytes_, static_cast<hipStream_t>(stream))
  GRAM_DISPATCH_M(spr_round_mt(m), RUN_CALL)
#undef RUN_CALL
  return rc;
}

extern "C" int spr_stats_gram_x32(const float *d_X, int64_t n_rows, int32_t m, int64_t ldx, int64_t row0,
                                  int64_t n_points, int32_t n_features, int32_t center, double *d_rowmean,
                                  void *d_workspace, size_t workspace_bytes_, void *stream) {
  int rc = check_args("spr_stats_gram_x32", d_X, n_rows, m, ldx, row0, n_points, n_features);
  if (rc != SPR_OK) return rc;
  SPR_REQUIRE(d_rowmean && d_workspace, SPR_E_INVALID, "spr_stats_gram_x32: NULL output/workspace");
  rc = SPR_E_UNSUPPORTED;
#define RUN_CALL(MTV)                                                                                \
  rc = launch<MTV>(d_X, n_rows, m, ldx, row0, n_points, n_features, center, d_rowmean, d_workspace, \
                   workspace_bytes_, static_cast<hipStream_t>(stream))
  GRAM_DISPATCH_M(spr_round_mt(m), RUN_CALL)
#undef RUN_CALL
  return rc;
}

extern "C" int spr_stats_gram_shifted_f64(const double *d_X, int64_t n_rows, int32_t m, int64_t ldx, int64_t row0,
                                          int64_t n_points, int32_t n_features, const double *d_shift,
                                          double *d_rowsum, void *d_workspace, size_t workspace_bytes_, void *stream) {
  int rc = check_args("spr_stats_gram_shifted_f64", d_X, n_rows, m, ldx, row0, n_points, n_features);
  if (rc != SPR_OK) return rc;
  SPR_REQUIRE(d_shift && d_rowsum && d_workspace, SPR_E_INVALID, "spr_stats_gram_shifted_f64: NULL pointer");
  rc = SPR_E_UNSUPPORTED;
#define RUN_CALL(MTV)                                                                                                    \
  rc = launch<MTV>(d_X, n_rows, m, ldx, row0, n_points, n_features, 2, const_cast<double *>(d_shift), d_workspace,       \
                   workspace_bytes_, static_cast<hipStream_t>(stream), d_rowsum)
  GRAM_DISPATCH_M(spr_round_mt(m), RUN_CALL)
#undef RUN_CALL
  return rc;
}

extern "C" int spr_stats_gram_shifted_x32(const float *d_X, int64_t n_rows, int32_t m, int64_t ldx, int64_t row0,
                                          int64_t n_points, int32_t n_features, const double *d_shift,
                                          double *d_rowsum, void *d_workspace, size_t workspace_bytes_, void *stream) {
  int rc = check_args("spr_stats_gram_shifted_x32", d_X, n_rows, m, ldx, row0, n_points, n_features);
  if (rc != SPR_OK) return rc;
  SPR_REQUIRE(d_shift && d_rowsum && d_workspace, SPR_E_INVALID, "spr_stats_gram_shifted_x32: NULL pointer");
  rc = SPR_E_UNSUPPORTED;
#define RUN_CALL(MTV)                                                                                                    \
  rc = launch<MTV>(d_X, n_rows, m, ldx, row0, n_points, n_features, 2, const_cast<double *>(d_shift), d_workspace,       \
                   workspace_bytes_, static_cast<hipStream_t>(stream), d_rowsum)
  GRAM_DISPATCH_M(spr_round_mt(m), RUN_CALL)
#undef RUN_CALL
  return rc;
}

extern "C" int spr_stats_gram_finalize_f64(int64_t n_rows, int32_t m, int64_t row0, int64_t n_points,
                                           int32_t n_features, const void *d_workspace, size_t workspace_bytes_,
                                           double *d_fstats, double *d_gram, int32_t ldg, int32_t origin,
                                           void *stream) {
  int rc = check_args("spr_stats_gram_finalize_f64", d_workspace, n_rows, m, m, row0, n_points, n_features);
  if (rc != SPR_OK) return rc;
  SPR_REQUIRE(d_fstats && d_gram, SPR_E_INVALID, "spr_stats_gram_finalize_f64: NULL output");
  SPR_REQUIRE(origin >= 0 && ldg >= origin + m, SPR_E_INVALID, "spr_stats_gram_finalize_f64: block (%d,%d)+%d outside ldg=%d",
              origin, origin, m, ldg);
  rc = SPR_E_UNSUPPORTED;
#define FIN_CALL(MTV)                                                                                 \
  rc = launch_finalize<MTV>(n_rows, m, row0, n_points, n_features, d_fstats, d_gram, ldg, origin, d_workspace, \
                            workspace_bytes_, static_cast<hipStream_t>(stream))
  GRAM_DISPATCH_M(spr_round_mt(m), FIN_CALL)
#undef FIN_CALL
  return rc;
}
```

Before: 1173.

## Split row panels equally across workgroups spanning feature boundaries

Adds an equal-split work plan where each workgroup takes a fixed quota of row panels that may cross one feature boundary, used by the gram-stats and projection kernels when m is at least 128 and rows are contiguous. The old per-feature proportional split could leave some workgroups holding more panels than others, and the new plan targets that load imbalance. The cost is a second segment pass per block, reworked slab and statistics slot indexing with a plan tag read by the finalize step, and more workspace. It is on by default and can be disabled with an environment variable.

```diff
diff --git a/include/spr_hip.h b/include/spr_hip.h
--- a/include/spr_hip.h
+++ b/include/spr_hip.h
@@ -35,6 +35,10 @@
                      void *fn_dormbr);
 
 size_t spr_stats_gram_workspace(int32_t m, int32_t n_features);
+int spr_stats_gram_equal_split(int32_t m, int64_t n_rows, int64_t row0, int64_t n_points, int32_t n_features,
+                               int32_t *panels_per_wg);
+int spr_project_equal_split(int32_t m, int32_t r, int64_t n_rows, int64_t row0, int64_t n_points,
+                            int32_t n_features, int32_t *panels_per_wg);
 int spr_stats_gram_f64(const double *d_X, int64_t n_rows, int32_t m, int64_t ldx,
                        int64_t row0, int64_t n_points, int32_t n_features, int32_t center,
                        double *d_rowmean, void *d_workspace, size_t workspace_bytes, void *stream);
diff --git a/openmeasure_amd/_lib.py b/openmeasure_amd/_lib.py
--- a/openmeasure_amd/_lib.py
+++ b/openmeasure_amd/_lib.py
@@ -29,6 +29,8 @@
     'spr_host_eig_top': (C.c_int, [_p, _i32, _i32, _p, _p, _p, _p, _p]),
     'spr_host_svd_top': (C.c_int, [_p, _i32, _i32, _p, _p, _p, _p, _p]),
     'spr_stats_gram_workspace': (_sz, [_i32, _i32]),
+    'spr_stats_gram_equal_split': (C.c_int, [_i32, _i64, _i64, _i64, _i32, _p]),
+    'spr_project_equal_split': (C.c_int, [_i32, _i32, _i64, _i64, _i64, _i32, _p]),
     'spr_stats_gram_f64': (C.c_int, [_p, _i64, _i32, _i64, _i64, _i64, _i32, _i32, _p, _p, _sz, _p]),
     'spr_stats_gram_finalize_f64': (C.c_int, [_i64, _i32, _i64, _i64, _i32, _p, _sz, _p, _p, _i32, _i32, _p]),
     'spr_stats_gram_shifted_f64': (C.c_int, [_p, _i64, _i32, _i64, _i64, _i64, _i32, _p, _p, _p, _sz, _p]),
diff --git a/openmeasure_amd/csrc/common.hpp b/openmeasure_amd/csrc/common.hpp
--- a/openmeasure_amd/csrc/common.hpp
+++ b/openmeasure_amd/csrc/common.hpp
@@ -40,63 +40,7 @@
 
 int spr_cached_cus();
 
-struct SegPlan {
-  int64_t row0, n_rows, n_points;
-  int32_t n_features;
-  int32_t total_wg;
-  int32_t chunk_rows;
-};
-
-__host__ __device__ inline void seg_range(const SegPlan &p, int f, int64_t &lo, int64_t &hi) {
-  int64_t glo = (int64_t)f * p.n_points, ghi = glo + p.n_points;
-  if (glo < p.row0) glo = p.row0;
-  if (ghi > p.row0 + p.n_rows) ghi = p.row0 + p.n_rows;
-  if (ghi < glo) ghi = glo;
-  lo = glo - p.row0;
-  hi = ghi - p.row0;
-}
-
-__host__ __device__ inline int seg_wgs(const SegPlan &p, int64_t rows) {
-  if (rows <= 0) return 0;
-  int64_t w = rows * (int64_t)p.total_wg / p.n_rows;
-  int64_t chunks = (rows + p.chunk_rows - 1) / p.chunk_rows;
-  if (w > chunks) w = chunks;
-  if (w < 1) w = 1;
-  return (int)w;
-}
-
-__host__ __device__ inline int seg_first_feature(const SegPlan &p) { return (int)(p.row0 / p.n_points); }
-__host__ __device__ inline int seg_last_feature(const SegPlan &p) {
-  int64_t f = (p.row0 + p.n_rows - 1) / p.n_points;
-  if (f > p.n_features - 1) f = p.n_features - 1;
-  return (int)f;
-}
-
-inline int seg_total_wgs(const SegPlan &p) {
-  int tot = 0;
-  for (int f = seg_first_feature(p); f <= seg_last_feature(p); ++f) {
-    int64_t lo, hi;
-    seg_range(p, f, lo, hi);
-    tot += seg_wgs(p, hi - lo);
-  }
-  return tot;
-}
-
-__device__ inline bool seg_locate(const SegPlan &p, int b, int &f, int &wl, int &wpf, int &base,
-                                  int64_t &lo, int64_t &hi) {
-  int acc = 0;
-  int f1 = seg_last_feature(p);
-  for (int ff = seg_first_feature(p); ff <= f1; ++ff) {
-    seg_range(p, ff, lo, hi);
-    int w = seg_wgs(p, hi - lo);
-    if (b < acc + w) {
-      f = ff; wl = b - acc; wpf = w; base = acc;
-      return true;
-    }
-    acc += w;
-  }
-  return false;
-}
+#include "segplan.hpp"
 
 template <int CTRL>
 __device__ inline double dpp_f64(double v) {
diff --git a/openmeasure_amd/csrc/launch.hpp b/openmeasure_amd/csrc/launch.hpp
--- a/openmeasure_amd/csrc/launch.hpp
+++ b/openmeasure_amd/csrc/launch.hpp
@@ -1,4 +1,6 @@
 #pragma once
+#include <stdlib.h>
+
 #include "common.hpp"
 
 inline int spr_cus_or_default() {
@@ -26,6 +28,13 @@
 }
 
 inline int spr_plan_grid(SegPlan &plan, int per_cu) { return spr_plan_grid(plan, per_cu, plan.chunk_rows); }
+
+inline bool spr_equal_split_enabled() {
+  const char *e = getenv("SPR_EQUAL_SPLIT");
+  return !(e && e[0] == '0');
+}
+
+inline bool spr_plan_equal(const SegPlan &plan) { return spr_equal_split_enabled() && eq_applicable(plan); }
 
 constexpr int spr_panel_per_cu(int mtr) { return mtr <= 1 ? 6 : mtr == 2 ? 4 : mtr == 3 ? 3 : mtr == 4 ? 2 : 1; }
 
diff --git a/openmeasure_amd/csrc/project_ws.hip b/openmeasure_amd/csrc/project_ws.hip
--- a/openmeasure_amd/csrc/project_ws.hip
+++ b/openmeasure_amd/csrc/project_ws.hip
@@ -47,17 +47,12 @@
 }
 
 template <int MT, int RT, int VEC, typename TX, typename TU, bool NRM>
-__global__ __launch_bounds__(WS_WAVES * 64) void project_ws_kernel(
-    const TX *__restrict__ X, int64_t ldx, int m, int center_i, SegPlan plan, const double *__restrict__ inv_scale,
-    const double *__restrict__ rowmean, const double *__restrict__ W, int r, TU *__restrict__ Ur, int64_t ldu,
-    double *__restrict__ nrm2) {
+__device__ __forceinline__ void ws_segment(
+    const TX *__restrict__ X, int64_t ldx, int m, int center_i, int f, int64_t lo, int64_t hi, int wl, int wpf,
+    const double *__restrict__ inv_scale, const double *__restrict__ rowmean, const double *__restrict__ W, int r,
+    TU *__restrict__ Ur, int64_t ldu, double *__restrict__ nrm2, double *__restrict__ Wl) {
   constexpr int K = 16 * MT, NJ = MT;
   constexpr int NC = WsLds<RT>::NC, LDW = WsLds<RT>::LDW;
-  __shared__ double Wl[K * LDW];
-
-  int f, wl, wpf, base;
-  int64_t lo, hi;
-  if (!seg_locate(plan, blockIdx.x, f, wl, wpf, base, lo, hi)) return;
 
   const int lane = threadIdx.x & 63;
   const int wave = __builtin_amdgcn_readfirstlane(threadIdx.x >> 6);
@@ -172,6 +167,29 @@
       }
     }
     c = cn;
+  }
+}
+
+template <int MT, int RT, int VEC, typename TX, typename TU, bool NRM, bool EQ>
+__global__ __launch_bounds__(WS_WAVES * 64) void project_ws_kernel(
+    const TX *__restrict__ X, int64_t ldx, int m, int center_i, SegPlan plan, const double *__restrict__ inv_scale,
+    const double *__restrict__ rowmean, const double *__restrict__ W, int r, TU *__restrict__ Ur, int64_t ldu,
+    double *__restrict__ nrm2) {
+  __shared__ double Wl[16 * MT * WsLds<RT>::LDW];
+  if constexpr (EQ) {
+    EqSeg seg[2];
+    const int nseg = eq_locate(plan, blockIdx.x, seg);
+#pragma nounroll
+    for (int s = 0; s < nseg; ++s) {
+      if (s) __syncthreads();
+      ws_segment<MT, RT, VEC, TX, TU, NRM>(X, ldx, m, center_i, s ? seg[1].f : seg[0].f, s ? seg[1].lo : seg[0].lo,
+                                           s ? seg[1].hi : seg[0].hi, 0, 1, inv_scale, rowmean, W, r, Ur, ldu, nrm2, Wl);
+    }
+  } else {
+    int f, wl, wpf, base;
+    int64_t lo, hi;
+    if (!seg_locate(plan, blockIdx.x, f, wl, wpf, base, lo, hi)) return;
+    ws_segment<MT, RT, VEC, TX, TU, NRM>(X, ldx, m, center_i, f, lo, hi, wl, wpf, inv_scale, rowmean, W, r, Ur, ldu, nrm2, Wl);
   }
 }
 
@@ -184,14 +202,29 @@
   const int grid = spr_plan_grid(plan, MT <= 4 ? narrow_per_cu : 1);
   const bool vec = (m == 16 * MT) && spr_rows_aligned16(X, sizeof(TX) * ldx);
   if (!vec) return SPR_E_UNSUPPORTED;
-  if (nrm2)
-    hipLaunchKernelGGL((project_ws_kernel<MT, RT, 1, TX, TU, true>), dim3(grid), dim3(WS_WAVES * 64), 0, st, X, ldx, (int)m,
-                       center, plan, inv_scale, rowmean, W, (int)r, Ur, ldu, nrm2);
-  else
-    hipLaunchKernelGGL((project_ws_kernel<MT, RT, 1, TX, TU, false>), dim3(grid), dim3(WS_WAVES * 64), 0, st, X, ldx, (int)m,
-                       center, plan, inv_scale, rowmean, W, (int)r, Ur, ldu, nrm2);
+#define WS_LAUNCH(NRMV, EQV, GRID)                                                                                          \
+  hipLaunchKernelGGL((project_ws_kernel<MT, RT, 1, TX, TU, NRMV, EQV>), dim3(GRID), dim3(WS_WAVES * 64), 0, st, X, ldx, (int)m, \
+                     center, plan, inv_scale, rowmean, W, (int)r, Ur, ldu, nrm2)
+  if constexpr (MT >= 8) {
+    if (ldx == m && spr_plan_equal(plan)) {
+      const int egrid = eq_grid(plan);
+      if (nrm2) WS_LAUNCH(true, true, egrid);
+      else WS_LAUNCH(false, true, egrid);
+      SPR_LAUNCH_CHECK();
+      return SPR_OK;
+    }
+  }
+  if (nrm2) WS_LAUNCH(true, false, grid);
+  else WS_LAUNCH(false, false, grid);
+#undef WS_LAUNCH
   SPR_LAUNCH_CHECK();
   return SPR_OK;
+}
+
+int32_t ws_equal_split(int64_t n_rows, int64_t row0, int64_t n_points, int32_t n_features) {
+  SegPlan plan = spr_make_plan(row0, n_rows, n_points, n_features, WS_ROWS);
+  spr_plan_grid(plan, 1);
+  return spr_plan_equal(plan) ? (int32_t)eq_quota(plan) : 0;
 }
 
 }
@@ -220,6 +253,20 @@
   return SPR_E_UNSUPPORTED;
 }
 
+extern "C" int spr_project_equal_split(int32_t m, int32_t r, int64_t n_rows, int64_t row0, int64_t n_points, int32_t n_features,
+                                       int32_t *panels_per_wg) {
+  SPR_REQUIRE(m > 0 && r > 0 && n_rows > 0, SPR_E_INVALID, "spr_project_equal_split: bad shape n_rows=%lld m=%d r=%d",
+              (long long)n_rows, m, r);
+  SPR_REQUIRE_LAYOUT("spr_project_equal_split", row0, n_rows, n_points, n_features);
+  SPR_REQUIRE(panels_per_wg != nullptr, SPR_E_INVALID, "spr_project_equal_split: NULL output");
+  bool fits = r <= 64 && m == 256;
+#ifndef PROJ_WS_LAB
+  fits = r <= 64 && (m == 128 || m == 192 || m == 256);
+#endif
+  *panels_per_wg = fits ? ws_equal_split(n_rows, row0, n_points, n_features) : 0;
+  return SPR_OK;
+}
+
 template int spr_project_ws<double, double>(const double *, int64_t, int32_t, int64_t, int64_t, int64_t, int32_t, int32_t,
                                             const double *, const double *, const double *, int32_t, double *, int64_t,
                                             int32_t, double *, hipStream_t);
diff --git a/openmeasure_amd/csrc/segplan.hpp b/openmeasure_amd/csrc/segplan.hpp
--- /dev/null
+++ b/openmeasure_amd/csrc/segplan.hpp
@@ -0,0 +1,156 @@
+#pragma once
+#include <stdint.h>
+
+#if defined(__HIPCC__)
+#define SPR_HD __host__ __device__
+#define SPR_DEV __device__
+#else
+#define SPR_HD
+#define SPR_DEV
+#endif
+
+struct SegPlan {
+  int64_t row0, n_rows, n_points;
+  int32_t n_features;
+  int32_t total_wg;
+  int32_t chunk_rows;
+};
+
+SPR_HD inline void seg_range(const SegPlan &p, int f, int64_t &lo, int64_t &hi) {
+  int64_t glo = (int64_t)f * p.n_points, ghi = glo + p.n_points;
+  if (glo < p.row0) glo = p.row0;
+  if (ghi > p.row0 + p.n_rows) ghi = p.row0 + p.n_rows;
+  if (ghi < glo) ghi = glo;
+  lo = glo - p.row0;
+  hi = ghi - p.row0;
+}
+
+SPR_HD inline int seg_wgs(const SegPlan &p, int64_t rows) {
+  if (rows <= 0) return 0;
+  int64_t w = rows * (int64_t)p.total_wg / p.n_rows;
+  int64_t chunks = (rows + p.chunk_rows - 1) / p.chunk_rows;
+  if (w > chunks) w = chunks;
+  if (w < 1) w = 1;
+  return (int)w;
+}
+
+SPR_HD inline int seg_first_feature(const SegPlan &p) { return (int)(p.row0 / p.n_points); }
+SPR_HD inline int seg_last_feature(const SegPlan &p) {
+  int64_t f = (p.row0 + p.n_rows - 1) / p.n_points;
+  if (f > p.n_features - 1) f = p.n_features - 1;
+  return (int)f;
+}
+
+inline int seg_total_wgs(const SegPlan &p) {
+  int tot = 0;
+  for (int f = seg_first_feature(p); f <= seg_last_feature(p); ++f) {
+    int64_t lo, hi;
+    seg_range(p, f, lo, hi);
+    tot += seg_wgs(p, hi - lo);
+  }
+  return tot;
+}
+
+SPR_DEV inline bool seg_locate(const SegPlan &p, int b, int &f, int &wl, int &wpf, int &base,
+                               int64_t &lo, int64_t &hi) {
+  int acc = 0;
+  int f1 = seg_last_feature(p);
+  for (int ff = seg_first_feature(p); ff <= f1; ++ff) {
+    seg_range(p, ff, lo, hi);
+    int w = seg_wgs(p, hi - lo);
+    if (b < acc + w) {
+      f = ff; wl = b - acc; wpf = w; base = acc;
+      return true;
+    }
+    acc += w;
+  }
+  return false;
+}
+
+struct EqSeg {
+  int32_t f;
+  int64_t lo, hi;
+};
+
+SPR_HD inline int64_t seg_panels(const SegPlan &p, int f) {
+  int64_t lo, hi;
+  seg_range(p, f, lo, hi);
+  return (hi - lo + p.chunk_rows - 1) / p.chunk_rows;
+}
+
+SPR_HD inline int64_t eq_total_panels(const SegPlan &p) {
+  int64_t tot = 0;
+  const int f1 = seg_last_feature(p);
+  for (int f = seg_first_feature(p); f <= f1; ++f) tot += seg_panels(p, f);
+  return tot;
+}
+
+SPR_HD inline int64_t eq_quota(const SegPlan &p) {
+  const int64_t tot = eq_total_panels(p);
+  return (p.total_wg > 0 && tot > 0) ? (tot + p.total_wg - 1) / p.total_wg : 0;
+}
+
+SPR_HD inline int64_t seg_max_share(const SegPlan &p) {
+  int64_t worst = 0;
+  const int f1 = seg_last_feature(p);
+  for (int f = seg_first_feature(p); f <= f1; ++f) {
+    int64_t lo, hi;
+    seg_range(p, f, lo, hi);
+    const int w = seg_wgs(p, hi - lo);
+    if (w > 0) {
+      const int64_t share = (seg_panels(p, f) + w - 1) / w;
+      if (share > worst) worst = share;
+    }
+  }
+  return worst;
+}
+
+SPR_HD inline bool eq_applicable(const SegPlan &p) {
+  const int f0 = seg_first_feature(p), f1 = seg_last_feature(p);
+  if (p.total_wg < 1 || p.chunk_rows < 1 || f1 <= f0) return false;
+  const int64_t q = eq_quota(p);
+  if (q < 1) return false;
+  for (int f = f0; f <= f1; ++f)
+    if (seg_panels(p, f) < q) return false;
+  return q < seg_max_share(p);
+}
+
+SPR_HD inline int eq_grid(const SegPlan &p) {
+  const int64_t q = eq_quota(p);
+  return q > 0 ? (int)((eq_total_panels(p) + q - 1) / q) : 0;
+}
+
+SPR_HD inline int eq_locate(const SegPlan &p, int b, EqSeg s[2]) {
+  const int64_t q = eq_quota(p);
+  const int64_t first = (int64_t)b * q, last = first + q;
+  int n = 0;
+  int64_t pre = 0;
+  const int f1 = seg_last_feature(p);
+  for (int f = seg_first_feature(p); f <= f1 && n < 2 && pre < last; ++f) {
+    int64_t lo, hi;
+    seg_range(p, f, lo, hi);
+    const int64_t np = (hi - lo + p.chunk_rows - 1) / p.chunk_rows;
+    const int64_t a = first > pre ? first : pre, z = last < pre + np ? last : pre + np;
+    if (a < z) {
+      const int64_t end = lo + (z - pre) * p.chunk_rows;
+      const EqSeg t = {f, lo + (a - pre) * p.chunk_rows, end < hi ? end : hi};
+      if (n == 0) s[0] = t;
+      else s[1] = t;
+      ++n;
+    }
+    pre += np;
+  }
+  return n;
+}
+
+SPR_HD inline void eq_contributors(const SegPlan &p, int f, int &b0, int &nb, int &slot0) {
+  const int64_t q = eq_quota(p);
+  int64_t pre = 0;
+  for (int ff = seg_first_feature(p); ff < f; ++ff) pre += seg_panels(p, ff);
+  const int64_t np = seg_panels(p, f);
+  b0 = 0; nb = 0; slot0 = 0;
+  if (q < 1 || np < 1) return;
+  b0 = (int)(pre / q);
+  nb = (int)((pre + np - 1) / q) - b0 + 1;
+  slot0 = ((int64_t)b0 * q < pre) ? 1 : 0;
+}
diff --git a/openmeasure_amd/csrc/stats_gram.hip b/openmeasure_amd/csrc/stats_gram.hip
--- a/openmeasure_amd/csrc/stats_gram.hip
+++ b/openmeasure_amd/csrc/stats_gram.hip
@@ -215,7 +215,8 @@
 template <int MT, int U, typename TX, bool EXT, bool SUMS>
 __device__ inline void gram_wave_own(const TX *__restrict__ X, int64_t ldx, int64_t lo, int64_t hi, int wl, int wpf, int ks,
                                      int wave, int lane, double *__restrict__ lds0, double *__restrict__ lds1,
-                                     double *__restrict__ rowmean, double *__restrict__ slab, double *__restrict__ rowsum) {
+                                     double *__restrict__ rowmean, double *__restrict__ slab, double *__restrict__ rowsum,
+                                     int slot) {
   using S = GramShape<MT>;
   using C = GramCfg<MT>;
   constexpr int R = C::R, KS = C::KS, NW = C::NW, MP = S::MP, T = S::T;
@@ -305,7 +306,7 @@
     cn = c2;
     nrow0 = n2row0;
   }
-  double *sp = slab + ((int64_t)blockIdx.x * KS + ks) * T * 256 + lane;
+  double *sp = slab + ((int64_t)slot * KS + ks) * T * 256 + lane;
 #pragma unroll
   for (int j = 0; j < NA; ++j) {
     double *tp = sp + (int64_t)tri_index(MT, RA, RA + j) * 256;
@@ -318,7 +319,7 @@
   }
 }
 
-template <int MT, typename TX, bool EXT, bool SUMS>
+template <int MT, typename TX, bool EXT, bool SUMS, bool EQ>
 __global__ __launch_bounds__(GramCfg<MT>::NW * 64) void stats_gram_own_kernel(
     const TX *__restrict__ X, int64_t ldx, SegPlan plan, double *__restrict__ rowmean, double *__restrict__ slab,
     double *__restrict__ rowsum) {
@@ -326,9 +327,18 @@
   using C = GramCfg<MT>;
   constexpr int NU = S::NU;
   __shared__ double lds[2][C::R * S::MP];
-  int f, wl, wpf, base;
-  int64_t lo, hi;
-  if (!seg_locate(plan, blockIdx.x, f, wl, wpf, base, lo, hi)) return;
+  int f, wl, wpf, base, nseg = 1;
+  int64_t lo, hi, lo1 = 0, hi1 = 0;
+  if constexpr (EQ) {
+    EqSeg seg[2];
+    nseg = eq_locate(plan, blockIdx.x, seg);
+    if (nseg == 0) return;
+    wl = 0; wpf = 1;
+    lo = seg[0].lo; hi = seg[0].hi;
+    if (nseg > 1) { lo1 = seg[1].lo; hi1 = seg[1].hi; }
+  } else {
+    if (!seg_locate(plan, blockIdx.x, f, wl, wpf, base, lo, hi)) return;
+  }
   const int lane = threadIdx.x & 63;
   const int wave = __builtin_amdgcn_readfirstlane(threadIdx.x >> 6);
   const int ks = wave / NU;
@@ -336,21 +346,38 @@
 #define GRAM_UNIT(UV)                                                                                          \
   case UV:                                                                                                     \
     if constexpr (UV < NU)                                                                                     \
-      gram_wave_own<MT, UV, TX, EXT, SUMS>(X, ldx, lo, hi, wl, wpf, ks, wave, lane, lds[0], lds[1], rowmean, slab, rowsum); \
+      gram_wave_own<MT, UV, TX, EXT, SUMS>(X, ldx, slo, shi, wl, wpf, ks, wave, lane, lds[0], lds[1], rowmean, slab, rowsum, slot); \
     break;
-  switch (unit) {
-    GRAM_UNIT(0) GRAM_UNIT(1) GRAM_UNIT(2) GRAM_UNIT(3) GRAM_UNIT(4) GRAM_UNIT(5) GRAM_UNIT(6) GRAM_UNIT(7)
-    default: break;
+  if constexpr (EQ) {
+#pragma nounroll
+    for (int s = 0; s < nseg; ++s) {
+      const int64_t slo = s ? lo1 : lo, shi = s ? hi1 : hi;
+      const int slot = 2 * (int)blockIdx.x + s;
+      if (s) __syncthreads();
+      switch (unit) {
+        GRAM_UNIT(0) GRAM_UNIT(1) GRAM_UNIT(2) GRAM_UNIT(3) GRAM_UNIT(4) GRAM_UNIT(5) GRAM_UNIT(6) GRAM_UNIT(7)
+        default: break;
+      }
+    }
+  } else {
+    const int64_t slo = lo, shi = hi;
+    const int slot = (int)blockIdx.x;
+    switch (unit) {
+      GRAM_UNIT(0) GRAM_UNIT(1) GRAM_UNIT(2) GRAM_UNIT(3) GRAM_UNIT(4) GRAM_UNIT(5) GRAM_UNIT(6) GRAM_UNIT(7)
+      default: break;
+    }
   }
 #undef GRAM_UNIT
 }
 
 constexpr int RS_THREADS = 1024;
 __global__ __launch_bounds__(RS_THREADS) void gram_rowmean_stats_kernel(const double *__restrict__ rowmean, SegPlan plan,
-                                                                        int slots_per_wg, double *__restrict__ stat_part) {
+                                                                        int slots_per_wg, double *__restrict__ stat_part,
+                                                                        int *__restrict__ plan_tag) {
   __shared__ double sn[RS_THREADS / 64], smu[RS_THREADS / 64], sm2[RS_THREADS / 64];
   int f, wl, wpf, base;
   int64_t lo, hi;
+  if (blockIdx.x == 0 && threadIdx.x == 0) *plan_tag = 0;
   if (!seg_locate(plan, blockIdx.x, f, wl, wpf, base, lo, hi)) return;
   const int lane = threadIdx.x & 63, wave = threadIdx.x >> 6;
   RowStats st;
@@ -376,6 +403,44 @@
     q[0] = n; q[1] = mu; q[2] = m2;
   }
   for (int e = 3 + threadIdx.x; e < slots_per_wg * 3; e += RS_THREADS) q[e] = 0.0;
+}
+
+__global__ __launch_bounds__(RS_THREADS) void gram_rowmean_stats_eq_kernel(const double *__restrict__ rowmean, SegPlan plan,
+                                                                           int slots_per_wg, double *__restrict__ stat_part,
+                                                                           int *__restrict__ plan_tag) {
+  __shared__ double sn[RS_THREADS / 64], smu[RS_THREADS / 64], sm2[RS_THREADS / 64];
+  EqSeg seg[2];
+  if (blockIdx.x == 0 && threadIdx.x == 0) *plan_tag = 1;
+  const int nseg = eq_locate(plan, blockIdx.x, seg);
+  if (nseg == 0) return;
+  const int lane = threadIdx.x & 63, wave = threadIdx.x >> 6;
+  double *q = stat_part + (int64_t)blockIdx.x * slots_per_wg * 3;
+  for (int s = 0; s < nseg; ++s) {
+    const int64_t lo = s ? seg[1].lo : seg[0].lo, hi = s ? seg[1].hi : seg[0].hi;
+    RowStats st;
+    st.init();
+    int64_t row = lo + threadIdx.x;
+    for (; row + 3 * RS_THREADS < hi; row += 4 * RS_THREADS) {
+      const double a = rowmean[row], b = rowmean[row + RS_THREADS], c = rowmean[row + 2 * RS_THREADS],
+                   d = rowmean[row + 3 * RS_THREADS];
+      st.push(a, true); st.push(b, true); st.push(c, true); st.push(d, true);
+    }
+    for (; row < hi; row += RS_THREADS) st.push(rowmean[row], true);
+    double n = st.cnt, mu = st.mean(), m2 = st.m2();
+    for (int o = 32; o > 0; o >>= 1) {
+      const double on = __shfl_down(n, o, 64), om = __shfl_down(mu, o, 64), os = __shfl_down(m2, o, 64);
+      chan_merge(n, mu, m2, on, om, os);
+    }
+    if (s) __syncthreads();
+    if (lane == 0) { sn[wave] = n; smu[wave] = mu; sm2[wave] = m2; }
+    __syncthreads();
+    if (threadIdx.x == 0) {
+      n = 0.0; mu = 0.0; m2 = 0.0;
+      for (int w = 0; w < RS_THREADS / 64; ++w) chan_merge(n, mu, m2, sn[w], smu[w], sm2[w]);
+      q[3 * s] = n; q[3 * s + 1] = mu; q[3 * s + 2] = m2;
+    }
+  }
+  for (int e = 3 * nseg + threadIdx.x; e < slots_per_wg * 3; e += RS_THREADS) q[e] = 0.0;
 }
 
 template <int MT, int VEC, typename TX>
@@ -411,14 +476,18 @@
 template <int MT>
 __global__ __launch_bounds__(1024) void gram_finalize_kernel(
     const double *__restrict__ slab, const double *__restrict__ stat_part, int m, SegPlan plan,
-    int slots_per_wg, double *__restrict__ gram, double *__restrict__ fstats, int ldg, int origin) {
+    int slots_per_wg, double *__restrict__ gram, double *__restrict__ fstats, int ldg, int origin,
+    const int *__restrict__ plan_tag) {
   constexpr int T = GramShape<MT>::T;
   constexpr int KS = GramOut<MT>::KSO;
   __shared__ double red[4][256];
   const int f = blockIdx.y;
   const int tile = blockIdx.x;
-  int base = 0, wpf = 0;
-  {
+  const bool eq = (MT >= 8) && *plan_tag == 1;
+  int base = 0, wpf = 0, slot0 = 0;
+  if (eq) {
+    eq_contributors(plan, f, base, wpf, slot0);
+  } else {
     int acc = 0;
     const int f0 = seg_first_feature(plan), f1 = seg_last_feature(plan);
     for (int ff = f0; ff <= f1; ++ff) {
@@ -433,17 +502,32 @@
   tile_coords<MT>(tile, ti, tj);
   const int e = threadIdx.x & 255, g = threadIdx.x >> 8;
   const int np = wpf * KS;
-  const double *sp = slab + ((int64_t)base * KS * T + tile) * 256 + e;
   const int64_t stride = (int64_t)T * 256;
   double s0 = 0.0, s1 = 0.0, s2 = 0.0, s3 = 0.0;
   int p = g;
-  for (; p + 12 < np; p += 16) {
-    s0 += sp[p * stride];
-    s1 += sp[(p + 4) * stride];
-    s2 += sp[(p + 8) * stride];
-    s3 += sp[(p + 12) * stride];
-  }
-  for (; p < np; p += 4) s0 += sp[p * stride];
+  if (eq) {
+    const double *sp = slab + (int64_t)tile * 256 + e;
+    auto at = [&](int pp) {
+      const int w = pp / KS;
+      return ((int64_t)(2 * (base + w) + (w == 0 ? slot0 : 0)) * KS + pp % KS) * stride;
+    };
+    for (; p + 12 < np; p += 16) {
+      s0 += sp[at(p)];
+      s1 += sp[at(p + 4)];
+      s2 += sp[at(p + 8)];
+      s3 += sp[at(p + 12)];
+    }
+    for (; p < np; p += 4) s0 += sp[at(p)];
+  } else {
+    const double *sp = slab + ((int64_t)base * KS * T + tile) * 256 + e;
+    for (; p + 12 < np; p += 16) {
+      s0 += sp[p * stride];
+      s1 += sp[(p + 4) * stride];
+      s2 += sp[(p + 8) * stride];
+      s3 += sp[(p + 12) * stride];
+    }
+    for (; p < np; p += 4) s0 += sp[p * stride];
+  }
   red[g][e] = (s0 + s1) + (s2 + s3);
   __syncthreads();
   if (g == 0) {
@@ -460,8 +544,15 @@
     __syncthreads();
     double n = 0.0, mu = 0.0, m2 = 0.0;
     const double *q = stat_part + (int64_t)base * slots_per_wg * 3;
-    const int tot_slots = wpf * slots_per_wg;
-    for (int pp = threadIdx.x; pp < tot_slots; pp += 1024) chan_merge(n, mu, m2, q[3 * pp], q[3 * pp + 1], q[3 * pp + 2]);
+    if (eq) {
+      for (int pp = threadIdx.x; pp < wpf; pp += 1024) {
+        const double *t = q + ((int64_t)pp * slots_per_wg + (pp == 0 ? slot0 : 0)) * 3;
+        chan_merge(n, mu, m2, t[0], t[1], t[2]);
+      }
+    } else {
+      const int tot_slots = wpf * slots_per_wg;
+      for (int pp = threadIdx.x; pp < tot_slots; pp += 1024) chan_merge(n, mu, m2, q[3 * pp], q[3 * pp + 1], q[3 * pp + 2]);
+    }
     double *sn = &red[0][0], *smu = &red[1][0], *sm2 = &red[2][0];
     for (int o = 32; o > 0; o >>= 1) {
       const double on = __shfl_down(n, o, 64), om = __shfl_down(mu, o, 64), os = __shfl_down(m2, o, 64);
@@ -501,12 +592,28 @@
 }
 
 template <int MT>
-size_t workspace_bytes(int32_t n_features) {
+struct GramWs {
   using RT = RowTile<MT, GramCfg<MT>::R, GramShape<MT>::MP, GramCfg<MT>::NW, GramCfg<MT>::LPRMAX>;
-  const int64_t max_grid = (int64_t)occupancy_wgs<MT>() + n_features;
-  return (size_t)max_grid * GramCfg<MT>::KS * GramShape<MT>::T * 256 * sizeof(double) +
-         (size_t)max_grid * RT::ROWS_PER_IT * 3 * sizeof(double);
-}
+  static_assert(RT::ROWS_PER_IT >= 2, "a block of the equal plan keeps two statistics triples");
+  int64_t max_grid, slab_slots;
+  explicit GramWs(int32_t n_features) {
+    const int64_t occ = occupancy_wgs<MT>();
+    max_grid = occ + n_features;
+    slab_slots = (MT >= 8 && 2 * occ > max_grid) ? 2 * occ : max_grid;
+  }
+  size_t slab_doubles() const { return (size_t)slab_slots * GramCfg<MT>::KS * GramShape<MT>::T * 256; }
+  size_t stat_doubles() const { return (size_t)max_grid * RT::ROWS_PER_IT * 3; }
+  size_t bytes() const { return (slab_doubles() + stat_doubles()) * sizeof(double) + (MT >= 8 ? 16 : 0); }
+  double *slab(void *ws) const { return static_cast<double *>(ws); }
+  double *stat_part(void *ws) const { return slab(ws) + slab_doubles(); }
+  int *plan_tag(void *ws) const { return MT >= 8 ? reinterpret_cast<int *>(stat_part(ws) + stat_doubles()) : nullptr; }
+};
+
+template <int MT>
+size_t workspace_bytes(int32_t n_features) { return GramWs<MT>(n_features).bytes(); }
+
+template <int MT>
+bool equal_plan(const SegPlan &plan) { return MT >= 8 && spr_plan_equal(plan); }
 
 template <int MT, typename TX>
 int launch(const TX *X, int64_t n_rows, int32_t m, int64_t ldx, int64_t row0, int64_t n_points,
@@ -517,10 +624,12 @@
   SPR_REQUIRE(!rowsum || center == 2, SPR_E_INVALID, "spr_stats_gram: row sums are an output of centre mode 2 only");
   SegPlan plan = make_plan<MT>(n_rows, row0, n_points, n_features);
   const int grid = seg_total_wgs(plan);
-  const int64_t max_grid = (int64_t)occupancy_wgs<MT>() + n_features;
+  const GramWs<MT> lay(n_features);
+  const int64_t max_grid = lay.max_grid;
   SPR_REQUIRE(grid >= 1 && grid <= max_grid, SPR_E_INVALID, "spr_stats_gram_f64: bad grid %d", grid);
-  double *slab = static_cast<double *>(ws);
-  double *stat_part = slab + (size_t)max_grid * GramCfg<MT>::KS * GramShape<MT>::T * 256;
+  double *slab = lay.slab(ws);
+  double *stat_part = lay.stat_part(ws);
+  int *plan_tag = lay.plan_tag(ws);
   const int lm = spr_load_mode(spr_pair_aligned(X, m, ldx), m, MT);
 #define SG_LAUNCH(LM)                                                                                         \
   hipLaunchKernelGGL((stats_gram_kernel<MT, LM, TX>), dim3(grid), dim3(GramCfg<MT>::NW * 64), 0, st, X, ldx, (int)m, \
@@ -529,22 +638,40 @@
   static const bool own_on = [] { const char *e = getenv("SPR_GRAM_OWN"); return !(e && e[0] == '0'); }();
   if (MT >= 8 && lm == 2 && (center == 1 || center == 2) && own_on && spr_rows_aligned16(X, sizeof(TX) * ldx)) {
     if constexpr (MT >= 8) {
+      if (ldx == m && equal_plan<MT>(plan)) {
+        const int egrid = eq_grid(plan);
+        SPR_REQUIRE(egrid >= 1 && 2 * (int64_t)egrid <= lay.slab_slots && egrid <= max_grid, SPR_E_INVALID,
+                    "spr_stats_gram_f64: bad grid %d", egrid);
+#define SG_OWN_EQ(EXTV, SUMSV)                                                                                         \
+  hipLaunchKernelGGL((stats_gram_own_kernel<MT, TX, EXTV, SUMSV, true>), dim3(egrid), dim3(GramCfg<MT>::NW * 64), 0, st, X, ldx, \
+                     plan, rowmean, slab, rowsum)
+        if (center == 1) SG_OWN_EQ(false, false);
+        else if (!rowsum) SG_OWN_EQ(true, false);
+        else SG_OWN_EQ(true, true);
+#undef SG_OWN_EQ
+        SPR_LAUNCH_CHECK();
+        hipLaunchKernelGGL(gram_rowmean_stats_eq_kernel, dim3(egrid), dim3(RS_THREADS), 0, st, rowmean, plan,
+                           (int)RTL::ROWS_PER_IT, stat_part, plan_tag);
+        SPR_LAUNCH_CHECK();
+        return SPR_OK;
+      }
       if (center == 1)
-        hipLaunchKernelGGL((stats_gram_own_kernel<MT, TX, false, false>), dim3(grid), dim3(GramCfg<MT>::NW * 64), 0, st, X, ldx,
+        hipLaunchKernelGGL((stats_gram_own_kernel<MT, TX, false, false, false>), dim3(grid), dim3(GramCfg<MT>::NW * 64), 0, st, X, ldx,
                            plan, rowmean, slab, rowsum);
       else if (!rowsum)
-        hipLaunchKernelGGL((stats_gram_own_kernel<MT, TX, true, false>), dim3(grid), dim3(GramCfg<MT>::NW * 64), 0, st, X, ldx,
+        hipLaunchKernelGGL((stats_gram_own_kernel<MT, TX, true, false, false>), dim3(grid), dim3(GramCfg<MT>::NW * 64), 0, st, X, ldx,
                            plan, rowmean, slab, rowsum);
       else
-        hipLaunchKernelGGL((stats_gram_own_kernel<MT, TX, true, true>), dim3(grid), dim3(GramCfg<MT>::NW * 64), 0, st, X, ldx,
+        hipLaunchKernelGGL((stats_gram_own_kernel<MT, TX, true, true, false>), dim3(grid), dim3(GramCfg<MT>::NW * 64), 0, st, X, ldx,
                            plan, rowmean, slab, rowsum);
       SPR_LAUNCH_CHECK();
       hipLaunchKernelGGL(gram_rowmean_stats_kernel, dim3(grid), dim3(RS_THREADS), 0, st, rowmean, plan, (int)RTL::ROWS_PER_IT,
-                         stat_part);
+                         stat_part, plan_tag);
       SPR_LAUNCH_CHECK();
       return SPR_OK;
     }
   }
+  if (plan_tag) SPR_HIP_TRY(hipMemsetAsync(plan_tag, 0, sizeof(int), st));
   if (lm == 2) SG_LAUNCH(2);
   else if (lm == 1) SG_LAUNCH(1);
   else SG_LAUNCH(0);
@@ -561,11 +688,13 @@
   SPR_REQUIRE(ws_bytes >= workspace_bytes<MT>(n_features), SPR_E_WORKSPACE,
               "spr_stats_gram_finalize_f64: workspace %zu < %zu", ws_bytes, workspace_bytes<MT>(n_features));
   SegPlan plan = make_plan<MT>(n_rows, row0, n_points, n_features);
-  const int64_t max_grid = (int64_t)occupancy_wgs<MT>() + n_features;
-  const double *slab = static_cast<const double *>(ws);
-  const double *stat_part = slab + (size_t)max_grid * GramCfg<MT>::KS * GramShape<MT>::T * 256;
+  const GramWs<MT> lay(n_features);
+  void *wsm = const_cast<void *>(ws);
+  const double *slab = lay.slab(wsm);
+  const double *stat_part = lay.stat_part(wsm);
   hipLaunchKernelGGL(gram_finalize_kernel<MT>, dim3(GramShape<MT>::T, n_features), dim3(1024), 0, st, slab,
-                     stat_part, (int)m, plan, (int)RT::ROWS_PER_IT, gram, fstats, ldg, origin);
+                     stat_part, (int)m, plan, (int)RT::ROWS_PER_IT, gram, fstats, ldg, origin,
+                     (const int *)lay.plan_tag(wsm));
   SPR_LAUNCH_CHECK();
   return SPR_OK;
 }
@@ -605,6 +734,23 @@
   GRAM_DISPATCH_M(spr_round_mt(m), WS_CALL)
 #undef WS_CALL
   return out;
+}
+
+extern "C" int spr_stats_gram_equal_split(int32_t m, int64_t n_rows, int64_t row0, int64_t n_points, int32_t n_features,
+                                          int32_t *panels_per_wg) {
+  int rc = check_args("spr_stats_gram_equal_split", &m, n_rows, m, m, row0, n_points, n_features);
+  if (rc != SPR_OK) return rc;
+  SPR_REQUIRE(panels_per_wg != nullptr, SPR_E_INVALID, "spr_stats_gram_equal_split: NULL output");
+  int32_t out = 0;
+#define EQ_CALL(MTV)                                                          \
+  if (m == 16 * MTV) {                                                        \
+    const SegPlan plan = make_plan<MTV>(n_rows, row0, n_points, n_features);  \
+    out = equal_plan<MTV>(plan) ? (int32_t)eq_quota(plan) : 0;                \
+  }
+  GRAM_DISPATCH_M(spr_round_mt(m), EQ_CALL)
+#undef EQ_CALL
+  *panels_per_wg = out;
+  return SPR_OK;
 }
 
 extern "C" int spr_stats_gram_f64(const double *d_X, int64_t n_rows, int32_t m, int64_t ldx, int64_t row0,
```

New measurement: 1182 (median of 6 runs). Within noise of the previous version (+0.8%).
